# GAMES-UChile/mogptk

Hardware: AMD Instinct MI355X
Metric: log-marginal-likelihood+grad evals/sec, MOSM C=4 N=8192; 1/2/4/8 GPU (higher is better)
Workload: dtype f64

## Files before the change

### mogptk_amd/csrc/exact.hip

```cpp
#include "mogp_model.h"
#include <cstdlib>
#include <limits>

using namespace mogp;

static int wait_stream(hipStream_t st) {
    static const bool spin = !(std::getenv("MOGP_SPIN_WAIT") && std::atoi(std::getenv("MOGP_SPIN_WAIT")) == 0);
    if (!spin) { HIP_TRY(hipStreamSynchronize(st)); return 0; }
    for (;;) {
        const hipError_t e = hipStreamQuery(st);
        if (e == hipSuccess) return 0;
        if (e != hipErrorNotReady) return hip_fail(e, "hipStreamQuery", __FILE__, __LINE__);
    }
}

static hipEvent_t prof_event(mogp_model* m, int idx) {
    if (!m->profiling) return nullptr;
    while ((int)m->ev.size() <= idx) { hipEvent_t e; if (hipEventCreate(&e) != hipSuccess) return nullptr; m->ev.push_back(e); }
    return m->ev[idx];
}

static void kinv_block_ranges(mogp_model* m) {
    std::vector<int> blk;
    tile_blocks(m->sx.off, m->C, blk);
// ... 40 lines not shown
    for (int i = 0; i < nb; ++i) {
        for (int j = 0; j <= i; ++j) {
            if (!need[(size_t)i * nb + j]) continue;
            GemmTask a;
            a.a_off = (int64_t)i * MOGP_TILE; a.b_off = (int64_t)j * MOGP_TILE; a.c_off = (int64_t)i * MOGP_TILE * ld + (int64_t)j * MOGP_TILE;
            a.kt = 4 * MOGP_TILE / 16; a.pad = i + 1;
            acc.push_back(a);
            GemmTask l;
            l.a_off = (int64_t)i * MOGP_TILE * ld + (int64_t)i * MOGP_TILE; l.b_off = (int64_t)i * MOGP_TILE * ld + (int64_t)j * MOGP_TILE;
            l.c_off = a.c_off; l.kt = (int)((ld - (int64_t)i * MOGP_TILE) / 16); l.pad = 0;
            lau.push_back(l);
        }
        prefix[i + 1] = (int)acc.size();
    }
    const double frac = (double)acc.size() / ((double)nb * (nb + 1) / 2);
    m->kinv_fraction = frac;
    if (frac > 0.85) return 0;
    const bool same = acc.size() == m->kinv_acc_tasks.size() && (acc.empty() || std::memcmp(acc.data(), m->kinv_acc_tasks.data(), acc.size() * sizeof(GemmTask)) == 0);
    if (!same || m->d_kinv_acc.n < acc.size()) {
        int rc;
        if ((rc = m->d_kinv_acc.ensure(std::max<size_t>(acc.size(), 1)))) return rc;
        if ((rc = m->d_kinv_lauum.ensure(std::max<size_t>(lau.size(), 1)))) return rc;
        HIP_TRY(hipMemcpyAsync(m->d_kinv_acc.p, acc.data(), acc.size() * sizeof(GemmTask), hipMemcpyHostToDevice, m->st));
        HIP_TRY(hipMemcpyAsync(m->d_kinv_lauum.p, lau.data(), lau.size() * sizeof(GemmTask), hipMemcpyHostToDevice, m->st));
        HIP_TRY(hipStreamSynchronize(m->st));
        m->kinv_acc_tasks.swap(acc); m->kinv_lauum_tasks.swap(lau);
    }
    m->kinv_prefix.swap(prefix);
    m->kinv_sparse = true;
    return 0;
}

static int pin_ensure(mogp_model* m, size_t n) {
    if (n <= m->h_pin_n) return 0;
    if (m->h_pin) { hipError_t e = hipHostFree(m->h_pin); (void)e; m->h_pin = nullptr; m->h_pin_n = 0; }
    HIP_TRY(hipHostMalloc(reinterpret_cast<void**>(&m->h_pin), n * sizeof(double), hipHostMallocDefault));
    m->h_pin_n = n;
    return 0;
}
struct PinLayout {
    size_t nzz, logdet = 0, zz, info, moments, diagG, pivots, total, score, mu, var, fold_info;
    PinLayout(int nb, int64_t Npad, int C, int T, int Wt) : nzz((size_t)((Npad + 3) / 4)) {
        zz = (size_t)nb; info = zz + nzz; moments = info + 1; diagG = moments + (size_t)(C * (C + 1) / 2) * T * Wt; pivots = diagG + C; total = pivots + 2;
        score = total; mu = score + 1; var = mu + (size_t)Npad; fold_info = var + (size_t)Npad;
    }
    explicit PinLayout(const mogp_model* m) : PinLayout(m->nb, m->Npad, m->C, m->T, m->Wt) {}
    size_t held_out_total(bool folds) const { return fold_info + (folds ? 1 : 0); }
};

namespace mogp {
int begin_call(mogp_model* m, int64_t* info, bool one_gpu) {
    m->mean_w = nullptr;
    if (int rc = use_device(m->ctx)) return rc;
    if (info) *info = 0;
    if (one_gpu) one_gpu_call(m);
    return 0;
}

int exact_begin(mogp_model* m, const double* noise_var, const double* data_var, double jitter, GramArgs& ga, double& jabs) {
    const int C = m->C;
    const int64_t N = m->N, Npad = m->Npad;
    if (m->T <= 0) return fail(MOGP_EINVAL, "mogp_model_set_terms must be called before an evaluation");
    if (!noise_var) return fail(MOGP_EINVAL, "noise_var is null");
    { int r__ = ensure_system(m); if (r__) return r__; }
    m->have_W = m->have_Kinv = false;
    m->gemm_ev_used = 0; m->gemm_launches = 0; m->gemm_flops = 0.0;

    double dsum = 0.0;
    if (!m->point_diag.empty()) {
        for (int c = 0; c < C; ++c)
            for (int k = m->sx.off[c]; k < m->sx.off[c + 1]; ++k) dsum += m->point_diag[k] + noise_var[c];
    } else if (m->radial && m->point_kinds) {
        dsum = table_diag_points(m, m->sx);
        for (int c = 0; c < C; ++c) dsum += (double)(m->sx.off[c + 1] - m->sx.off[c]) * noise_var[c];
    } else
    for (int c = 0; c < C; ++c) dsum += (double)(m->sx.off[c + 1] - m->sx.off[c]) * (table_diag(m, c) + noise_var[c]);
    if (data_var) {
        std::vector<double> dv(Npad, 0.0);
        for (int64_t pos = 0; pos < N; ++pos) { dv[pos] = data_var[m->sx.perm[pos]]; dsum += dv[pos]; }
        { int r__ = m->d_dvar.ensure(Npad); if (r__) return r__; }
        HIP_TRY(hipMemcpyAsync(m->d_dvar.p, dv.data(), Npad * sizeof(double), hipMemcpyHostToDevice, m->st));
    }
    jabs = jitter * dsum / (double)N;
    HIP_TRY(hipMemcpyAsync(m->d_noise.p, noise_var, C * sizeof(double), hipMemcpyHostToDevice, m->st));
    static const unsigned long long big = std::numeric_limits<unsigned long long>::max();
    HIP_TRY(hipMemcpyAsync(m->d_info.p, &big, sizeof(big), hipMemcpyHostToDevice, m->st));
    int rc;
    if ((rc = mark(m, 0))) return rc;
    ga = GramArgs{};
    ga.tiles = m->d_tiles.p; ga.xr = m->d_x.p; ga.xc = m->d_x.p; ga.ldxr = ga.ldxc = Npad; ga.nrows = ga.ncols = N;
    if ((rc = m->ph_xx.prepare(m->sx.off, m->sx.off, C, m->T, Npad, Npad, m->st, ga.ph))) return rc;
    ga.table = m->d_table.p; ga.T = m->T; ga.D = m->D; ga.C = C; ga.W = m->Wt;
    ga.out = m->k.A.p; ga.ldo = Npad; ga.noise = m->d_noise.p; ga.dvar = data_var ? m->d_dvar.p : nullptr;
    ga.jitter_abs = jabs; ga.mirror = 0;
    if (m->radial) { ga.kind = m->d_kind.p; ga.shape = m->d_shape.p; }
    return 0;
}
}

namespace mogp { int chain_fallback(mogp_model* m) {
    if (m->flow_ran) {
        m->no_flow = true; m->flow_ran = false;
        m->flow_timeouts++;
        m->flow_retry_at = m->n_fact + m->flow_backoff;
        m->flow_backoff = std::min(m->flow_backoff * 4, 16384);
        for (hipStream_t q : {m->st, m->st2, m->st3, m->st4, m->ctx->st5, m->st_priv}) if (q) HIP_TRY(hipStreamSynchronize(q));
        static bool said_flow = false;
        if (!said_flow) {
            said_flow = true;
            unsigned code = 0;
            if (m->k.flow_flags.p && m->k.flow_cur && m->k.flow_cur->base_err > 0) { hipError_t e = hipMemcpy(&code, m->k.flow_flags.p + m->k.flow_cur->base_err, sizeof(code), hipMemcpyDeviceToHost); (void)e; }
            fprintf(stderr, "mogp: the dataflow kernel timed out (wait 0x%x; GPU shared with another process?); using the stream schedule for the next %d evaluations (said once)\n", code, (int)(m->flow_retry_at - m->n_fact));
            fprintf(stderr, "mogp: the host enqueued that evaluation in %.0f us (longest so far %.0f us)\n", m->flow_enqueue_us, m->flow_enqueue_us_max);
        }
        if (std::getenv("MOGP_FLOW_DEBUG")) { fprintf(stderr, "mogp: dataflow time-out %d of this model\n", m->flow_timeouts); flow_debug_dump(m); }
        return 0;
    }
    if (m->no_chain) return fail(MOGP_EHIP, "chain kernel: a hand-off timed out although the model is on the launch-per-step chain");
    m->no_chain = true;
    for (hipStream_t q : {m->st, m->st2, m->st3, m->st4, m->ctx->st5, m->st_priv}) if (q) HIP_TRY(hipStreamSynchronize(q));
    static bool said = false;
    if (!said) { said = true; fprintf(stderr, "mogp: the persistent chain kernel timed out (GPU shared with another process?); using the launch-per-step chain\n"); }
    return 0;
} }

template <typename F> static int retry_on_streams(mogp_model* m, int rc, F again) {
    if (rc != MOGP_RETRY_NO_CHAIN) return rc;
    if ((rc = chain_fallback(m))) return rc;
    return again();
}

namespace mogp { int report_not_pd(unsigned long long hinfo, int64_t* info) {
    if (info) *info = (int64_t)hinfo;
    return fail(MOGP_ENOTPD, "linalg.cholesky: The factorization could not be completed because the input is not "
                             "positive-definite (the leading minor of order " + std::to_string(hinfo) + " is not positive-definite).");
} }

static int factorize_finish(mogp_model* m, const GramArgs& ga, double* lml, int64_t* info) {
    const int64_t N = m->N, Npad = m->Npad;
    const PinLayout pl(m);
    const unsigned long long big = std::numeric_limits<unsigned long long>::max();
    unsigned long long hinfo = 0;
    std::memcpy(&hinfo, m->h_pin + pl.info, sizeof(hinfo));
    int rc;
    if (hinfo == MOGP_INFO_CHAIN_TIMEOUT) return MOGP_RETRY_NO_CHAIN;
    if (hinfo != big) {
        if (info) *info = (int64_t)hinfo;
        int flag = 0;
        HIP_TRY(hipMemsetAsync(m->d_flag.p, 0, sizeof(int), m->st));
        if ((rc = launch_gram(ga, (int)m->tiles.size(), m->st, m->radial ? m->gate_kinds : 0))) return rc;
        if ((rc = launch_nonfinite_scan(m->k.A.p, Npad, N, m->d_flag.p, m->st))) return rc;
        HIP_TRY(hipMemcpyAsync(&flag, m->d_flag.p, sizeof(int), hipMemcpyDeviceToHost, m->st));
        HIP_TRY(hipStreamSynchronize(m->st));
        if (flag & 1) return fail(MOGP_ENONFINITE, "linalg.cholesky: kernel matrix has NaNs!");
        if (flag & 2) return fail(MOGP_ENONFINITE, "linalg.cholesky: kernel matrix has infinities!");
        return report_not_pd(hinfo, info);
    }
    m->pivot_min = m->h_pin[pl.pivots]; m->pivot_max = m->h_pin[pl.pivots + 1];
    double logdet = 0.0, zz = 0.0;
    for (int i = 0; i < m->nb; ++i) logdet += m->h_pin[pl.logdet + i];
    for (size_t i = 0; i < pl.nzz; ++i) zz += m->h_pin[pl.zz + i];
    if (lml) *lml = -0.5 * (double)N * std::log(2.0 * M_PI) - logdet - 0.5 * zz;
    m->have_W = !m->factor_only && !m->accurate_ran;
    return 0;
}

struct FactorPlan {
    enum Schedule { Fused, Phases, FactorOnly } schedule = Phases;
    bool defer = false;
    bool want_inverse = true;
    bool refine = false;
};

static int factorize(mogp_model* m, const double* noise_var, const double* data_var, double jitter, const FactorPlan& plan,
                     double* lml, double* jitter_abs, int64_t* info, GramArgs* ga_out = nullptr) {
    const bool fuse_inverse = plan.schedule == FactorPlan::Fused, factor_only = plan.schedule == FactorPlan::FactorOnly;
    const int64_t N = m->N, Npad = m->Npad;
    GramArgs ga{};
    double jabs = 0.0;
    int rc = exact_begin(m, noise_var, data_var, jitter, ga, jabs);
    if (rc) return rc;
    if (jitter_abs) *jitter_abs = jabs;
    m->n_fact++;
    if (m->no_flow && m->n_fact >= m->flow_retry_at) m->no_flow = false;
    m->factor_only = factor_only;
    ga.ev0 = prof_event(m, 7); ga.ev1 = prof_event(m, 8);
    m->strip.attach(ga);
    const bool split = fuse_inverse && flow_enabled(m, m->k) && !m->tiles_head.empty() && !m->tiles_tail.empty() && m->st2;
    if (split) {
        GramArgs gh = ga, gt = ga;
        gh.tiles = m->d_tiles_head.p; m->strip_head.attach(gh); gh.ev1 = nullptr;
        gt.tiles = m->d_tiles_tail.p; m->strip_tail.attach(gt); gt.ev0 = nullptr; gt.phases_ready = 1;
        if ((rc = launch_gram(gh, (int)m->tiles_head.size(), m->st, m->radial ? m->gate_kinds : 0))) return rc;
        if ((rc = launch_pad_identity(m->k.A.p, Npad, N, Npad, m->st))) return rc;
        if (!m->gram_ev) HIP_TRY(hipEventCreateWithFlags(&m->gram_ev, hipEventDisableTiming));
        HIP_TRY(hipEventRecord(m->gram_ev, m->st));
        HIP_TRY(hipStreamWaitEvent(m->st2, m->gram_ev, 0));
        if ((rc = launch_gram(gt, (int)m->tiles_tail.size(), m->st2, m->radial ? m->gate_kinds : 0))) return rc;
        if (!m->gram_tail_ev) HIP_TRY(hipEventCreateWithFlags(&m->gram_tail_ev, hipEventDisableTiming));
        HIP_TRY(hipEventRecord(m->gram_tail_ev, m->st2));
        m->k.tail_ready = m->gram_tail_ev;
    } else {
        if ((rc = launch_gram(ga, (int)m->tiles.size(), m->st, m->radial ? m->gate_kinds : 0))) return rc;
        if ((rc = launch_pad_identity(m->k.A.p, Npad, N, Npad, m->st))) return rc;
    }
    ga.ev0 = ga.ev1 = nullptr;
    if ((rc = mark(m, 1))) return rc;

    const PinLayout pl(m);
    if ((rc = pin_ensure(m, pl.total))) return rc;
    if ((rc = m->d_pivots.ensure(2))) return rc;
    if (m->accurate && (rc = m->acc_rhs.ensure((size_t)Npad * MOGP_TILE))) return rc;
    m->k.flow_used = false;
    m->flow_ran = false;
    m->k.want_vec = fuse_inverse;
    m->k.vec_y = m->d_y.p; m->k.vec_z = m->d_z.p; m->k.vec_zz = m->d_zz.p; m->k.vec_part = m->d_alpha.p + Npad;
    const bool accurate = m->accurate && plan.schedule == FactorPlan::Phases;
    m->accurate_ran = accurate;
    m->k.keep_L = m->k.refine_panels = plan.refine || accurate;
    if (factor_only && m->rhs_job && flow_enabled(m, m->k)) rc = spd_potri_flow(m, m->k, m->rhs_job);
    else rc = fuse_inverse ? spd_potri_fused(m, m->k) : spd_potrf(m, m->k);
    m->k.keep_L = m->k.refine_panels = false;
    m->k.want_vec = false; m->k.tail_ready = nullptr;
    if (rc) return rc;
    if ((rc = mark(m, 2))) return rc;
    if (accurate) {
        hipStream_t ms = (plan.want_inverse && m->st2u) ? m->st2u : m->st;
        if (plan.want_inverse) {
            if (ms != m->st) {
                while ((int)m->k.inv_ev.size() < 4) { hipEvent_t e; HIP_TRY(hipEventCreateWithFlags(&e, hipEventDisableTiming)); m->k.inv_ev.push_back(e); }
                HIP_TRY(hipEventRecord(m->k.inv_ev[0], m->st));
                HIP_TRY(hipStreamWaitEvent(ms, m->k.inv_ev[0], 0));
            }
            if ((rc = m->k.Wm.ensure((size_t)Npad * Npad))) return rc;
            HIP_TRY(hipMemsetAsync(m->k.Wm.p, 0, (size_t)Npad * Npad * sizeof(double), ms));
            if ((rc = launch_add_diag(m->k.Wm.p, Npad, Npad, 1.0, ms))) return rc;
            if ((rc = trsm_lower(m, m->k.A.p, Npad, m->nb, m->k.Wm.p, Npad, Npad, false, ms, true))) return rc;
            GemmArgs g{};
            g.A = m->k.Wm.p; g.lda = Npad; g.a_kmajor = 1; g.B = m->k.Wm.p; g.ldb = Npad; g.b_kmajor = 1;
            g.C = m->k.B.p; g.ldc = Npad; g.alpha = 1.0; g.beta = 0.0; g.mode = GM_LAUUM; g.mt = g.nt = m->nb; g.K = (int)Npad;
            if ((rc = gemm_call(m, g, gemm_flops(g, nullptr), ms))) return rc;
            if (ms != m->st) HIP_TRY(hipEventRecord(m->k.inv_ev[1], ms));
        }
        HIP_TRY(hipMemsetAsync(m->acc_rhs.p, 0, (size_t)Npad * MOGP_TILE * sizeof(double), m->st));
        if ((rc = launch_copy2d(m->acc_rhs.p, MOGP_TILE, m->d_y.p, 1, Npad, 1, 1.0, m->st))) return rc;
        if ((rc = trsm_lower(m, m->k.A.p, Npad, m->nb, m->acc_rhs.p, MOGP_TILE, MOGP_TILE, false))) return rc;
        if ((rc = launch_copy2d(m->d_z.p, 1, m->acc_rhs.p, MOGP_TILE, Npad, 1, 1.0, m->st))) return rc;
        HIP_TRY(hipMemsetAsync(m->d_zz.p, 0, pl.nzz * sizeof(double), m->st));
        if ((rc = launch_gemv_rows(m->d_z.p, Npad, 1, Npad, m->d_z.p, m->d_zz.p, m->st))) return rc;
        if ((rc = trsm_lower(m, m->k.A.p, Npad, m->nb, m->acc_rhs.p, MOGP_TILE, MOGP_TILE, true))) return rc;
        if ((rc = launch_copy2d(m->d_alpha.p, 1, m->acc_rhs.p, MOGP_TILE, Npad, 1, 1.0, m->st))) return rc;
        if (plan.want_inverse && ms != m->st) HIP_TRY(hipStreamWaitEvent(m->st, m->k.inv_ev[1], 0));
    } else if (plan.schedule == FactorPlan::Phases && (rc = spd_trtri(m, m->k))) return rc;
    if ((rc = mark(m, 3))) return rc;

    if (factor_only) {
        HIP_TRY(hipMemsetAsync(m->d_zz.p, 0, pl.nzz * sizeof(double), m->st));
    } else if (!accurate) {
        const double* Wp = fuse_inverse ? m->k.Wm.p : m->k.A.p;
        m->w_in_Wm = fuse_inverse;
        if (fuse_inverse && m->k.flow_used && m->k.vec_done) {
            if ((rc = launch_flow_alpha_sum(m->k, m->d_alpha.p, m->st))) return rc;
        } else {
            if ((rc = launch_trmv_lower(Wp, Npad, Npad, m->d_y.p, m->d_z.p, m->d_zz.p, m->st))) return rc;
            if ((rc = launch_trmv_lower_t(Wp, Npad, Npad, m->d_z.p, m->d_alpha.p, m->st))) return rc;
        }
    }
    if (fuse_inverse && (rc = spd_potri_fused_finish(m, m->k))) return rc;
    if ((rc = mark(m, 4))) return rc;
    {
        static const bool fault = std::getenv("MOGP_FLOW_FAULT") && std::atoi(std::getenv("MOGP_FLOW_FAULT")) != 0;
        static const unsigned long long timed_out = MOGP_INFO_CHAIN_TIMEOUT;
        if (fault && m->k.flow_used) HIP_TRY(hipMemcpyAsync(m->d_info.p, &timed_out, sizeof(timed_out), hipMemcpyHostToDevice, m->st));
    }

    const int nzz = (int)pl.nzz;
    if ((rc = launch_pivot_range(m->k.invd.p, N, m->d_pivots.p, m->st))) return rc;
    HIP_TRY(hipMemcpyAsync(m->h_pin + pl.pivots, m->d_pivots.p, 2 * sizeof(double), hipMemcpyDeviceToHost, m->st));
    HIP_TRY(hipMemcpyAsync(m->h_pin + pl.logdet, m->k.logdet.p, m->nb * sizeof(double), hipMemcpyDeviceToHost, m->st));
    constexpr int zz_piece = 2048;
    for (int o = 0; o < nzz; o += zz_piece)
        HIP_TRY(hipMemcpyAsync(m->h_pin + pl.zz + o, m->d_zz.p + o, std::min(zz_piece, nzz - o) * sizeof(double), hipMemcpyDeviceToHost, m->st));
    HIP_TRY(hipMemcpyAsync(m->h_pin + pl.info, m->d_info.p, sizeof(unsigned long long), hipMemcpyDeviceToHost, m->st));
    if (ga_out) *ga_out = ga;
    if (plan.defer) return 0;
    HIP_TRY(hipStreamSynchronize(m->st));
    return factorize_finish(m, ga, lml, info);
}

namespace mogp { void collect_timing(mogp_model* m, int last_mark) {
    if (!m->profiling) return;
    auto el = [&](int a, int b) { float t = 0.f; if (hipEventElapsedTime(&t, m->ev[a], m->ev[b]) != hipSuccess) t = 0.f; return (double)t; };
    std::fill(m->ms, m->ms + MOGP_ST_COUNT, 0.0);
    m->ms[MOGP_ST_GRAM] = el(0, 1);
    m->ms[MOGP_ST_POTRF] = el(1, 2);
    m->ms[MOGP_ST_TRTRI] = el(2, 3);
    m->ms[MOGP_ST_SOLVE] = el(3, 4);
    if (last_mark >= 6) { m->ms[MOGP_ST_LAUUM] = el(4, 5); m->ms[MOGP_ST_MOMENTS] = el(5, 6); }
    m->ms[MOGP_ST_TOTAL] = el(0, last_mark);
    if ((int)m->ev.size() > 8) m->ms[MOGP_ST_GRAM_KERNEL] = el(7, 8);
    if (last_mark >= 6 && (int)m->ev.size() > 10) m->ms[MOGP_ST_MOMENT_KERNEL] = el(9, 10);
    double gsum = 0.0;
    for (size_t i = 0; i + 1 < m->gemm_ev_used; i += 2) {
        float t = 0.f;
        if (hipEventElapsedTime(&t, m->gemm_ev[i], m->gemm_ev[i + 1]) == hipSuccess) gsum += t;
    }
    m->ms[MOGP_ST_GEMM_KERNEL] = gsum;
}

int moment_pass_device(mogp_model* m, const double* kinv, double ksign) {
    const int C = m->C, D = m->D, W = m->Wt, T = m->T, P = C * (C + 1) / 2;
    const int64_t Npad = m->Npad;
    const int rm = m->sh_n > 1 ? m->sh_n : 0;
    const bool own = m->sh_n > 1 && m->own_n == m->sh_n && m->own_rank == m->sh_rank;
    int rc;
    MomentArgs ma{};
    ma.tiles = own ? m->d_tiles_own.p : m->d_tiles.p; ma.ntiles = (int)(own ? m->tiles_own.size() : m->tiles.size());
    ma.x = m->d_x.p; ma.ldx = Npad; ma.nrows = ma.ncols = m->N;
    if ((rc = m->ph_xx.prepare(m->sx.off, m->sx.off, C, T, Npad, Npad, m->st, ma.ph))) return rc;
    ma.table = m->d_table.p; ma.T = T; ma.D = D; ma.C = C; ma.W = W; ma.kinv = kinv; ma.kinv_sign = ksign; ma.ld = Npad; ma.alpha = m->d_alpha.p;
    ma.row_mod = rm; ma.row_rem = m->sh_rank;
    if (m->radial) { ma.kind = m->d_kind.p; ma.shape = m->d_shape.p; }
    ma.partial = m->d_partial.p;
    ma.phases_ready = 1;
    ma.ev0 = prof_event(m, 9); ma.ev1 = prof_event(m, 10);
    if ((rc = launch_moments(ma, m->st, m->radial ? m->gate_kinds : 0))) return rc;
    if ((rc = launch_moment_reduce(m->d_partial.p, own ? m->d_pair_start_own.p : m->d_pair_start.p, P, T, W, D, m->d_moments.p, m->st))) return rc;
    if ((rc = launch_diagG(kinv, Npad, m->d_alpha.p, m->d_chan_off.p, C, m->d_diagG.p, m->st, ksign, rm, m->sh_rank))) return rc;
    if ((rc = mean_grad_enqueue(m, m->d_alpha.p, -1.0))) return rc;
    return mark(m, 6);
}

int moment_pass(mogp_model* m, const double* kinv, double ksign, double* moments, double* diagG) {
    const int C = m->C, W = m->Wt, T = m->T, P = C * (C + 1) / 2;
    int rc;
    if ((rc = moment_pass_device(m, kinv, ksign))) return rc;
    HIP_TRY(hipMemcpyAsync(moments, m->d_moments.p, (size_t)P * T * W * sizeof(double), hipMemcpyDeviceToHost, m->st));
    HIP_TRY(hipMemcpyAsync(diagG, m->d_diagG.p, C * sizeof(double), hipMemcpyDeviceToHost, m->st));
    HIP_TRY(hipStreamSynchronize(m->st));
    return 0;
}

int test_side(mogp_model* m, int64_t S, const double* Xs, const double* kss_diag, int64_t extra_rows, hipStream_t st, TestSide& ts, GramArgs& ga, int R, bool point_diag) {
    const int C = m->C, D = m->D;
    const int64_t Npad = m->Npad;
    SortedX& ss = ts.ss;
    int rc;
    if ((rc = sort_inputs(Xs, S, D, C, MOGP_TILE, ss))) return rc;
    const int64_t Spad = ts.Spad = ss.Mpad, Srow = R * Spad + extra_rows;
    std::vector<GTile> pt;
    build_rect_tiles(ss.off, m->sx.off, C, pt);
    ts.ntiles = (int)pt.size();
    if ((rc = m->d_xs.ensure((size_t)D * Spad))) return rc;
    if ((rc = m->d_Ksf.ensure((size_t)Srow * Npad))) return rc;
    if ((rc = m->d_mu.ensure((size_t)R * Spad))) return rc;
    if ((rc = m->d_kdiag.ensure((size_t)R * Spad))) return rc;
    if ((rc = m->d_ptiles.ensure(std::max<size_t>(pt.size(), 1)))) return rc;
    std::vector<double> kd((size_t)R * Spad, 0.0);
    const bool per_point = point_diag || m->Wt > 2 + 3 * D || (m->radial && m->point_kinds);
    for (int r = 0; r < R; ++r) {
        const double* kr = kss_diag + (size_t)r * (per_point ? S : C);
        for (int c = 0; c < C; ++c)
            for (int pos = ss.off[c]; pos < ss.off[c + 1]; ++pos) kd[(size_t)r * Spad + pos] = per_point ? kr[ss.perm[pos]] : kr[c];
    }
    HIP_TRY(hipMemcpyAsync(m->d_xs.p, ss.xs.data(), (size_t)D * Spad * sizeof(double), hipMemcpyHostToDevice, st));
    HIP_TRY(hipMemcpyAsync(m->d_kdiag.p, kd.data(), (size_t)R * Spad * sizeof(double), hipMemcpyHostToDevice, st));
    HIP_TRY(hipMemcpyAsync(m->d_ptiles.p, pt.data(), pt.size() * sizeof(GTile), hipMemcpyHostToDevice, st));
    HIP_TRY(hipMemsetAsync(m->d_Ksf.p, 0, (size_t)Srow * Npad * sizeof(double), st));
    ga = GramArgs{};
    ga.tiles = m->d_ptiles.p; ga.xr = m->d_xs.p; ga.ldxr = Spad; ga.xc = m->d_x.p; ga.ldxc = Npad; ga.nrows = S; ga.ncols = m->N;
    if ((rc = m->ph_sx.prepare(ss.off, m->sx.off, C, m->T, Spad, Npad, st, ga.ph))) return rc;
    ga.table = m->d_table.p; ga.T = m->T; ga.D = D; ga.C = C; ga.W = m->Wt; ga.out = m->d_Ksf.p; ga.ldo = Npad;
    ga.noise = nullptr; ga.dvar = nullptr; ga.jitter_abs = 0.0; ga.mirror = 0;
    if (m->radial) { ga.kind = m->d_kind.p; ga.shape = m->d_shape.p; }
    return 0;
}
}

static const std::string& grad_path_env() {
    static const std::string grad_path = []() { const char* e = std::getenv("MOGP_GRAD_PATH"); return std::string(e ? e : ""); }();
    return grad_path;
}

static int enqueue_inverse(mogp_model* m, const double* noise_var, const double* data_var, double jitter, bool inverse, bool banded,
                           double* lml, double* jitter_abs, int64_t* info, GramArgs& ga) {
    const std::string& grad_path = grad_path_env();
    int rc;
    if ((rc = ensure_system(m))) return rc;
    if ((rc = kinv_plan(m, inverse && banded && !m->accurate))) return rc;
    const int fused_max = flow_enabled(m, m->k) ? 112 : 80;
    const bool fused = inverse && !m->accurate && (grad_path == "fused" || (grad_path != "phases" && m->nb <= fused_max));
    FactorPlan plan;
    plan.schedule = fused ? FactorPlan::Fused : FactorPlan::Phases; plan.defer = inverse; plan.want_inverse = inverse;
    if ((rc = factorize(m, noise_var, data_var, jitter, plan, lml, jitter_abs, info, &ga))) return rc;
    if (!inverse) return 0;
    if (!fused && !m->accurate_ran && (rc = spd_lauum(m, m->k))) return rc;
    return mark(m, 5);
}

static int grad_enqueue(mogp_model* m, const PinLayout& pl) {
    HIP_TRY(hipMemcpyAsync(m->h_pin + pl.moments, m->d_moments.p, (pl.diagG - pl.moments) * sizeof(double), hipMemcpyDeviceToHost, m->st));
    HIP_TRY(hipMemcpyAsync(m->h_pin + pl.diagG, m->d_diagG.p, m->C * sizeof(double), hipMemcpyDeviceToHost, m->st));
    return 0;
}
static void grad_finish(mogp_model* m, const double* diagG, double* trG) {
    double tr = 0.0;
    for (int c = 0; c < m->C; ++c) tr += diagG[c];
    *trG = tr;
    mean_grad_collect(m);
    collect_timing(m, 6);
}
static void grad_collect(mogp_model* m, const PinLayout& pl, double* moments, double* diagG, double* trG) {
    std::memcpy(moments, m->h_pin + pl.moments, (pl.diagG - pl.moments) * sizeof(double));
    std::memcpy(diagG, m->h_pin + pl.diagG, m->C * sizeof(double));
    grad_finish(m, diagG, trG);
}

static int held_out_eval(mogp_model* m, const double* noise_var, const double* data_var, double jitter, int flags, const int32_t* fold, int64_t nfolds,
                         double* score, double* mu, double* var, double* moments, double* diagG, double* trG, double* jitter_abs, int64_t* info) {
    const bool grad = (flags & MOGP_EVAL_GRAD) != 0, folds = fold != nullptr;
    int rc;
    if ((rc = begin_call(m, info, true))) return rc;
    auto again = [&]() {
        return folds ? mogp_exact_cv(m, noise_var, data_var, jitter, flags, fold, nfolds, score, mu, var, moments, diagG, trG, jitter_abs, info)
                     : mogp_exact_loo(m, noise_var, data_var, jitter, flags, score, mu, var, moments, diagG, trG, jitter_abs, info);
    };
    if ((rc = ensure_system(m))) return rc;
    if ((rc = folds ? cv_workspace(m, fold, nfolds, grad) : loo_workspace(m, grad))) return rc;
    const PinLayout pl(m);
    if ((rc = pin_ensure(m, pl.held_out_total(folds)))) return rc;
    const int64_t N = m->N, Npad = m->Npad;
    GramArgs ga{};
    if ((rc = enqueue_inverse(m, noise_var, data_var, jitter, true, false, nullptr, jitter_abs, info, ga))) return retry_on_streams(m, rc, again);
    if ((rc = held_out_points(m, m->k.B.p, folds, grad))) return rc;
    if (grad) {
        m->have_W = false;
        if ((rc = held_out_adjoint(m, m->k.B.p, m->k.A.p, folds))) return rc;
        if ((rc = loo_moment_pass(m))) return rc;
        if ((rc = grad_enqueue(m, pl))) return rc;
    }
    const double* v = m->loo.vec.p;
    double* h = m->h_pin;
    HIP_TRY(hipMemcpyAsync(h + pl.score, v + LOO_SUM * Npad, sizeof(double), hipMemcpyDeviceToHost, m->st));
    HIP_TRY(hipMemcpyAsync(h + pl.mu, v + LOO_MU * Npad, N * sizeof(double), hipMemcpyDeviceToHost, m->st));
    HIP_TRY(hipMemcpyAsync(h + pl.var, v + LOO_VAR * Npad, N * sizeof(double), hipMemcpyDeviceToHost, m->st));
    if (folds) HIP_TRY(hipMemcpyAsync(h + pl.fold_info, m->d_info.p, sizeof(unsigned long long), hipMemcpyDeviceToHost, m->st));
    if ((rc = wait_stream(m->st))) return rc;
    if ((rc = factorize_finish(m, ga, nullptr, info))) return retry_on_streams(m, rc, again);
    if (grad) m->have_W = false;
    if (folds) {
        unsigned long long finfo = 0;
        std::memcpy(&finfo, h + pl.fold_info, sizeof(finfo));
        if (finfo != std::numeric_limits<unsigned long long>::max()) {
            if (info) *info = (int64_t)(finfo - 1) / 256;
            return fail(MOGP_ENOTPD, "mogp_exact_cv: the block of Kj^-1 over fold " + std::to_string((finfo - 1) / 256) + " is not positive definite (pivot " +
                                     std::to_string((finfo - 1) % 256 + 1) + " of its factorisation): Kj is too ill-conditioned for this fold");
        }
        for (int64_t pos = 0; pos < N; ++pos)
            if (m->cv.label[pos] < 0) h[pl.mu + pos] = h[pl.var + pos] = std::numeric_limits<double>::quiet_NaN();
    }
    *score = h[pl.score];
    scatter_by_perm(m->sx, h + pl.mu, mu);
    scatter_by_perm(m->sx, h + pl.var, var);
    m->have_Kinv = true;
    m->kinv_in_A = false;
    if (!grad) { collect_timing(m, 5); return MOGP_OK; }
    grad_collect(m, pl, moments, diagG, trG);
    return MOGP_OK;
}

extern "C" {

int mogp_exact_eval(mogp_model* m, const double* noise_var, const double* data_var, double jitter, int flags,
                    double* lml, double* moments, double* diagG, double* trG, double* jitter_abs, int64_t* info) {
    if (!m) return fail(MOGP_EINVAL, "mogp_exact_eval: model is null");
    int rc;
    if ((rc = begin_call(m, info, true))) return rc;
    const std::string& grad_path = grad_path_env();
    const bool sweep = grad_path == "sweep" && (flags & MOGP_EVAL_GRAD);
    const bool grad = (flags & MOGP_EVAL_GRAD) != 0;
    GramArgs ga{};
    auto again = [&]() { return mogp_exact_eval(m, noise_var, data_var, jitter, flags, lml, moments, diagG, trG, jitter_abs, info); };
    if (grad && (!moments || !diagG || !trG)) return fail(MOGP_EINVAL, "mogp_exact_eval: gradient outputs are null");
    if (sweep) {
        if ((rc = ensure_system(m))) return rc;
// ... 324 lines not shown
```

### mogptk_amd/csrc/flow.hip

```cpp
#include "mogp_model.h"
#include <unistd.h>
#include <chrono>
#include <set>

#include <cstdio>
#include <cstdlib>

namespace mogp {

typedef double d4_t __attribute__((ext_vector_type(4)));
typedef double d2_t __attribute__((ext_vector_type(2)));

#define FL_BK 16
#define FL_ROWK 18
#define FL_WTM 4
#define FL_WTN 2
#define FL_NWJ 4
#define FL_NWI 2
#define FL_NT 512
#define FL_COLK (MOGP_TILE + 16)
#define FL_OPER (MOGP_TILE * FL_ROWK)
#define FL_LDS_DOUBLES (2 * 2 * FL_OPER)
#define FL_LDS_BYTES (FL_LDS_DOUBLES * 8 + 16 + 3 * 64 * 4 + 16)
static_assert(MOGP_TILE * FL_ROWK == 16 * FL_COLK, "one LDS operand slot serves both layouts");
// ... 620 lines not shown
            vec.push_back(t);
        }
        for (int jg = 0; jg * 4 < k1(b); ++jg) {
            FlowTask t = mk(b, PH_APART, 32 | 1, nk(b));
            t.ar = (uint16_t)k0(b); t.br = (uint16_t)b; t.ac = (uint16_t)jg;
            dep(t, ZR(b), (unsigned)nk(b));
            vec.push_back(t);
        }
    }
    std::vector<const std::vector<FlowTask>*> order = {&q[Q_LOOK2], &q[Q_SEMI], &q[Q_INVCRIT], &vec};
    for (int d = 2; d < no + 3; ++d) {
        if (d < no && !into[d].empty()) order.push_back(&into[d]);
        if (d - 3 >= 0 && d - 3 < no && !trail[d - 3].empty()) order.push_back(&trail[d - 3]);
    }
    order.push_back(rhs_nt > 0 ? &rrest : &acc);
    for (size_t k = order.size(); k-- > 1;) if (order[k]->empty()) order.erase(order.begin() + (long)k);
    if ((int)order.size() > FLOW_MAXQ) {
        std::vector<FlowTask> rest;
        std::vector<const std::vector<FlowTask>*> tail(order.begin() + (FLOW_MAXQ - 2), order.end() - 1);
        for (auto* v : tail) rest.insert(rest.end(), v->begin(), v->end());
        std::stable_sort(rest.begin(), rest.end(), [](const FlowTask& x, const FlowTask& y) { return x.key < y.key; });
        p.folded = rest;
        order.erase(order.begin() + (FLOW_MAXQ - 2), order.end() - 1);
        order.insert(order.end() - 1, &p.folded);
    }
    p.nq = (int)order.size();
    for (int qi = 0; qi < p.nq; ++qi) {
        p.qbase[qi] = (int)p.tasks.size(); p.qsize[qi] = (int)order[qi]->size();
        p.tasks.insert(p.tasks.end(), order[qi]->begin(), order[qi]->end());
    }
    p.flops = 2.0 * MOGP_TILE * MOGP_TILE * FL_BK * tiles_k;
}

__global__ void k_alpha_sum(const double* __restrict__ part, int64_t npad, int no, int ob, double* __restrict__ out) {
    const int64_t col = (int64_t)blockIdx.x * blockDim.x + threadIdx.x;
    if (col >= npad) return;
    double s = 0.0;
    for (int r = (int)(col / MOGP_TILE) / ob; r < no; ++r) s += part[(int64_t)r * npad + col];
    out[col] = s;
}
int launch_flow_alpha_sum(const Spd& w, double* alpha, hipStream_t st) {
    const FlowPlan& p = w.flow_cur ? *w.flow_cur : w.flow;
    hipLaunchKernelGGL(k_alpha_sum, dim3((unsigned)((w.Npad + 255) / 256)), dim3(256), 0, st, w.vec_part, w.Npad, p.nouter, p.ob, alpha);
    HIP_TRY(hipGetLastError());
    return 0;
}

bool flow_enabled(const mogp_model* m, const Spd& w) {
    const char* eo = std::getenv("MOGP_FLOW");
    const char* en = std::getenv("MOGP_FLOW_MIN");
    const int on = eo ? std::atoi(eo) : 1, nmin = en ? std::atoi(en) : 8;
    if (!on || (m->no_flow && m->n_fact < m->flow_retry_at) || !chain_enabled(m) || !m->ctx->st_priv) return false;
    if (m->kinv_sparse && &w == &m->k) return false;
    return w.nb >= nmin && w.nb <= 0xfff0;
}

int spd_potri_flow(mogp_model* m, Spd& w, const FlowRhs* rhs) {
    const int nb = w.nb, ob = 4;
    const int64_t ld = w.Npad;
    int rc;
    const auto host_t0 = std::chrono::steady_clock::now();
    hipStream_t crit = m->st, priv = m->st_priv, bulk = m->st2;
    if (w.Wm.n < (size_t)ld * ld) {
        if ((rc = w.Wm.ensure((size_t)ld * ld))) return rc;
        HIP_TRY(hipMemsetAsync(w.Wm.p, 0, (size_t)ld * ld * sizeof(double), crit));
    }
    if ((rc = w.Lm.ensure((size_t)ld * ld))) return rc;
    if (!rhs && (rc = w.Wt.ensure((size_t)ld * ld))) return rc;
    const bool replay = m->replay_flow && !rhs && &w == &m->k;
    FlowPlan& plan = rhs ? w.flow_rhs : replay ? w.flow_replay : w.flow;
    DevBuf<FlowTask>& d_tasks = rhs ? w.flow_tasks_rhs : replay ? w.flow_tasks_replay : w.flow_tasks;
    DevBuf<int>& d_qmeta = rhs ? w.flow_qmeta_rhs : replay ? w.flow_qmeta_replay : w.flow_qmeta;
    const int rhs_nt = rhs ? rhs->nt : 0;
    if (plan.nb != nb || plan.ob != ob || plan.rhs_nt != rhs_nt) {
        flow_build(nb, ob, plan, rhs_nt, replay);
        if ((rc = d_tasks.ensure(plan.tasks.size()))) return rc;
        if ((rc = d_qmeta.ensure(2 * FLOW_MAXQ))) return rc;
        int qm[2 * FLOW_MAXQ] = {0};
        for (int q = 0; q < plan.nq; ++q) { qm[2 * q] = plan.qbase[q]; qm[2 * q + 1] = plan.qsize[q]; }
        HIP_TRY(hipStreamSynchronize(crit));
        HIP_TRY(dev_upload(d_tasks.p, plan.tasks.data(), plan.tasks.size() * sizeof(FlowTask)));
        HIP_TRY(dev_upload(d_qmeta.p, qm, sizeof(qm)));
    }
    if ((rc = w.flow_flags.ensure((size_t)plan.nflags))) return rc;
    if (!w.flow_diag.p) {
        if ((rc = w.flow_diag.ensure(FLOW_DIAG_WORDS))) return rc;
        HIP_TRY(hipMemsetAsync(w.flow_diag.p, 0, FLOW_DIAG_WORDS * sizeof(unsigned), crit));
    }
    w.flow_cur = &plan;
    const FlowPlan& p = plan;
    const int nouter = p.nouter;
    if ((rc = w.chain_flags.ensure((size_t)(nouter + 1) * MOGP_CHAIN_FLAGS))) return rc;
    HIP_TRY(hipMemsetAsync(w.chain_flags.p, 0, (size_t)(nouter + 1) * MOGP_CHAIN_FLAGS * sizeof(unsigned), crit));
    HIP_TRY(hipMemsetAsync(w.flow_flags.p, 0, (size_t)p.nflags * sizeof(unsigned), crit));
    if (replay) {
        std::vector<unsigned> preset((size_t)p.nflags, 0u);
        for (const FlowPlan::Chain& c : p.chain) preset[c.done_idx] = c.expect;
        HIP_TRY(hipMemcpyAsync(w.flow_flags.p, preset.data(), preset.size() * sizeof(unsigned), hipMemcpyHostToDevice, crit));
        HIP_TRY(hipStreamSynchronize(crit));
    }
    if (!rhs && w.want_vec && w.vec_zz) HIP_TRY(hipMemsetAsync(w.vec_zz, 0, (size_t)((ld + 3) / 4) * sizeof(double), crit));
    static const bool want_trace = std::getenv("MOGP_FLOW_TRACE") && std::atoi(std::getenv("MOGP_FLOW_TRACE")) != 0;
    if (want_trace) {
        if ((rc = w.flow_trace.ensure(FLOW_TRACE_W * p.tasks.size() + 4 * (size_t)nouter))) return rc;
        HIP_TRY(hipMemsetAsync(w.flow_trace.p, 0, w.flow_trace.n * sizeof(unsigned long long), crit));
    }
    while ((int)w.inv_ev.size() < 4) {
        hipEvent_t e;
        HIP_TRY(hipEventCreateWithFlags(&e, hipEventDisableTiming));
        w.inv_ev.push_back(e);
    }
    hipEvent_t start = w.inv_ev[0], e_flow = w.inv_ev[1], e_chain = w.inv_ev[2];
    HIP_TRY(hipEventRecord(start, crit));
    HIP_TRY(hipStreamWaitEvent(bulk, start, 0));
    HIP_TRY(hipStreamWaitEvent(priv, start, 0));

    static std::atomic<unsigned long long> attr_done{0ull};
    static std::atomic<unsigned long long> attr_done_dbg{0ull};
    { int r__ = set_max_dynamic_lds(reinterpret_cast<const void*>(k_flow<false>), FL_LDS_BYTES, attr_done); if (r__) return r__; }
    { int r__ = set_max_dynamic_lds(reinterpret_cast<const void*>(k_flow<true>), FL_LDS_BYTES, attr_done_dbg); if (r__) return r__; }
    static const int wg_per_cu = std::getenv("MOGP_FLOW_WGS") ? std::max(1, std::atoi(std::getenv("MOGP_FLOW_WGS"))) : 2;
    int cus = (m->ctx->ncu > 0 ? m->ctx->ncu : 256) - m->ctx->ncu_reserved;
    { static const int drop = std::getenv("MOGP_FLOW_DROP_CUS") ? std::atoi(std::getenv("MOGP_FLOW_DROP_CUS")) : 16;
      if (drop > 0 && drop < cus) cus -= drop; }
    FlowArgs g{};
    g.bA = w.A.p; g.bL = w.Lm.p; g.bWt = rhs ? rhs->T : w.Wt.p; g.bWm = w.Wm.p; g.bB = rhs ? rhs->X : w.B.p; g.ld = ld;
    g.tasks = d_tasks.p; g.qmeta = d_qmeta.p; g.flags = w.flow_flags.p;
    g.nq = p.nq; g.ncas = FLOW_NCAS; g.base_heads = p.base_heads; g.base_err = p.base_err; g.info = m->d_info.p;
    g.trace = want_trace ? w.flow_trace.p : nullptr;
    g.diag = w.flow_diag.p;
    static const bool want_post = std::getenv("MOGP_FLOW_DEBUG") && std::atoi(std::getenv("MOGP_FLOW_DEBUG")) != 0;
    if (want_post) {
        const size_t nwg = (size_t)wg_per_cu * ((size_t)cus + (size_t)m->ctx->ncu_reserved);
        if ((rc = w.flow_post.ensure(nwg * FLOW_POST_W))) return rc;
        HIP_TRY(hipMemsetAsync(w.flow_post.p, 0, w.flow_post.n * sizeof(unsigned), bulk));
        g.post = w.flow_post.p;
        if ((rc = w.flow_done.ensure(p.tasks.size()))) return rc;
        HIP_TRY(hipMemsetAsync(w.flow_done.p, 0, p.tasks.size(), bulk));
        g.done = w.flow_done.p;
    }
    g.npad = ld;
    { const char* e = std::getenv("MOGP_FLOW_REFILL"); g.refill = e ? std::atoi(e) : 0; }
    { const char* e = std::getenv("MOGP_FLOW_CLAIM1"); g.claim_one = e ? std::atoi(e) : 0; }
    { const char* e = std::getenv("MOGP_FLOW_NHI"); g.nhi = e ? std::atoi(e) : 0; }
    { const char* e = std::getenv("MOGP_FLOW_NAP"); g.nap_max = e ? (unsigned)std::max(0, std::atoi(e)) : 4u; }
    { const char* e = std::getenv("MOGP_FLOW_NAP_CALM"); g.nap_calm = e ? (unsigned)std::max(0, std::atoi(e)) : 0u; if (g.nap_calm < g.nap_max) g.nap_calm = g.nap_max; }
    w.vec_done = false;
    if (!rhs && w.want_vec && w.vec_y && w.vec_z && w.vec_zz && w.vec_part) {
        g.vy = w.vec_y; g.vz = w.vec_z; g.vzz = w.vec_zz; g.vpart = w.vec_part;
        w.vec_done = true;
    }
    hipEvent_t pe0 = nullptr, pe1 = nullptr;
    if (m->profiling) {
        if (m->gemm_ev_used + 2 > m->gemm_ev.size())
            for (int i = 0; i < 64; ++i) { hipEvent_t e; HIP_TRY(hipEventCreate(&e)); m->gemm_ev.push_back(e); }
        pe0 = m->gemm_ev[m->gemm_ev_used++]; pe1 = m->gemm_ev[m->gemm_ev_used++];
        HIP_TRY(hipEventRecord(pe0, bulk));
    }
    if (rhs && rhs->ready) HIP_TRY(hipStreamWaitEvent(bulk, rhs->ready, 0));
    const bool dbg_kernel = g.post != nullptr || g.trace != nullptr;
    static_assert(sizeof(FlowArgs) <= 512, "Spd::flow_args slots");
    if ((rc = w.flow_args.ensure(1024))) return rc;
    if (w.flow_args_h.size() != 2048) w.flow_args_h.assign(2048, (char)0xff);
    auto upload = [&](size_t slot, const FlowArgs& a, hipStream_t st) -> int {
        char* held = w.flow_args_h.data() + slot;
        char* fresh_ = w.flow_args_h.data() + 1024 + slot;
        std::memset(fresh_, 0, 512);
        std::memcpy(fresh_, &a, sizeof(a));
        if (std::memcmp(held, fresh_, 512) == 0) return 0;
        HIP_TRY(hipStreamSynchronize(st));
        HIP_TRY(dev_upload(w.flow_args.p + slot, fresh_, 512));
        std::memcpy(held, fresh_, 512);
        return 0;
    };
    if ((rc = upload(0, g, bulk))) return rc;
    const FlowArgs* d_g = reinterpret_cast<const FlowArgs*>(w.flow_args.p);
    FlowHot hot{};
    hot.bA = g.bA; hot.bL = g.bL; hot.bWt = g.bWt; hot.bWm = g.bWm; hot.bB = g.bB; hot.ld = g.ld; hot.tasks = g.tasks; hot.qmeta = g.qmeta; hot.flags = g.flags;
    hot.nq = g.nq; hot.ncas = g.ncas; hot.base_heads = g.base_heads; hot.base_err = g.base_err; hot.nap_max = g.nap_max; hot.nap_calm = g.nap_calm;
    if (dbg_kernel) hipLaunchKernelGGL(k_flow<true>, dim3(wg_per_cu * cus), dim3(FL_NT), FL_LDS_BYTES, bulk, d_g, hot);
    else hipLaunchKernelGGL(k_flow<false>, dim3(wg_per_cu * cus), dim3(FL_NT), FL_LDS_BYTES, bulk, d_g, hot);
    HIP_TRY(hipGetLastError());
    if (pe1) HIP_TRY(hipEventRecord(pe1, bulk));
    HIP_TRY(hipEventRecord(e_flow, bulk));
    m->gemm_launches += 1;
    m->gemm_flops += p.flops;

    unsigned* ferr = w.flow_flags.p + p.base_err;
    for (int kb = 0; kb < nouter && !replay; ++kb) {
        const int k0 = kb * ob, k1 = std::min(k0 + ob, nb), nk = k1 - k0, na = std::min(ob, nb - k1);
        const FlowPlan::Chain& pc = p.chain[kb];
        ChainFlow cf{};
        cf.done_flag = w.flow_flags.p + pc.done_idx; cf.write_through = 1;
        cf.trace = want_trace ? w.flow_trace.p + FLOW_TRACE_W * p.tasks.size() + 4 * (size_t)kb : nullptr;
        cf.diag = w.flow_diag.p;
        if ((rc = launch_chain(w.A.p, ld, k0, nk, w.invd.p, w.logdet.p, m->d_info.p, 0, w.Wm.p + (int64_t)k0 * MOGP_TILE * (ld + 1), ld,
                               w.chain_flags.p + (size_t)kb * MOGP_CHAIN_FLAGS, ferr, priv, &cf))) return rc;
        if (na <= 0) continue;
        GemmArgs t1{};
        t1.A = w.A.p + (int64_t)k1 * MOGP_TILE * ld + (int64_t)k0 * MOGP_TILE; t1.lda = ld; t1.a_kmajor = 0;
        t1.B = w.Wm.p + (int64_t)k0 * MOGP_TILE * (ld + 1); t1.ldb = ld; t1.b_kmajor = 0;
        t1.C = w.Lm.p + (int64_t)k1 * MOGP_TILE * ld + (int64_t)k0 * MOGP_TILE; t1.ldc = ld; t1.alpha = 1.0; t1.beta = 0.0;
        t1.mode = GM_KHI_J; t1.small = 1; t1.mt = 2 * na; t1.nt = nk; t1.K = nk * MOGP_TILE;
        t1.fl_flags = w.flow_flags.p; t1.fl_nwait = pc.t1_nwait;
        for (int k = 0; k < pc.t1_nwait; ++k) { t1.fl_widx[k] = pc.t1_widx[k]; t1.fl_wval[k] = pc.t1_wval[k]; }
        static const unsigned hook_spins = std::getenv("MOGP_FLOW_HOOK_SPINS") ? (unsigned)std::atoll(std::getenv("MOGP_FLOW_HOOK_SPINS")) : 0u;
        t1.fl_spins = hook_spins; t1.fl_diag = w.flow_diag.p;
        t1.fl_wt = 1; t1.fl_sig = 1; t1.fl_sig_base = pc.t1_sig_base; t1.fl_sig_shift = 1; t1.fl_err = ferr; t1.sk_info = m->d_info.p;
        if ((rc = launch_gemm(t1, priv))) return rc;
        if (kb == 0 && w.tail_ready) HIP_TRY(hipStreamWaitEvent(priv, w.tail_ready, 0));
        GemmArgs t2{};
        t2.A = t1.C; t2.lda = ld; t2.a_kmajor = 0; t2.B = t1.C; t2.ldb = ld; t2.b_kmajor = 0;
        t2.C = w.A.p + (int64_t)k1 * MOGP_TILE * (ld + 1); t2.ldc = ld; t2.alpha = -1.0; t2.beta = 1.0;
        t2.mode = GM_RECT_LOWER; t2.small = 2; t2.mt = 2 * na; t2.nt = 2 * na; t2.K = nk * MOGP_TILE;
        t2.fl_flags = w.flow_flags.p; t2.fl_nwait = pc.t2_wval ? 1 : 0; t2.fl_widx[0] = pc.t2_widx; t2.fl_wval[0] = pc.t2_wval;
        t2.fl_err = ferr; t2.sk_info = m->d_info.p; t2.fl_spins = hook_spins; t2.fl_diag = w.flow_diag.p;
        if ((rc = launch_gemm(t2, priv))) return rc;
        m->gemm_flops += gemm_flops(t1, nullptr) + gemm_flops(t2, nullptr);
    }
    static const bool tail_on = !(std::getenv("MOGP_FLOW_TAIL") && std::atoi(std::getenv("MOGP_FLOW_TAIL")) == 0);
    if (tail_on && m->ctx->ncu_reserved > 0 && !replay) {
        if (rhs && rhs->ready) HIP_TRY(hipStreamWaitEvent(priv, rhs->ready, 0));
        g.post_base = wg_per_cu * cus;
        if ((rc = upload(512, g, priv))) return rc;
        const FlowArgs* d_g2 = reinterpret_cast<const FlowArgs*>(w.flow_args.p + 512);
        if (dbg_kernel) hipLaunchKernelGGL(k_flow<true>, dim3(wg_per_cu * m->ctx->ncu_reserved), dim3(FL_NT), FL_LDS_BYTES, priv, d_g2, hot);
        else hipLaunchKernelGGL(k_flow<false>, dim3(wg_per_cu * m->ctx->ncu_reserved), dim3(FL_NT), FL_LDS_BYTES, priv, d_g2, hot);
        HIP_TRY(hipGetLastError());
    }
    HIP_TRY(hipEventRecord(e_chain, priv));
    HIP_TRY(hipStreamWaitEvent(crit, e_flow, 0));
    HIP_TRY(hipStreamWaitEvent(crit, e_chain, 0));
    w.fused_last_inv = nullptr; w.fused_last_wt = nullptr;
    w.flow_used = true;
    m->flow_ran = true;
    m->flow_enqueue_us = std::chrono::duration<double, std::micro>(std::chrono::steady_clock::now() - host_t0).count();
    m->flow_enqueue_us_max = std::max(m->flow_enqueue_us_max, m->flow_enqueue_us);
    { const char* e = std::getenv("MOGP_FLOW_DEBUG");
      if (e && std::atoi(e) == 2 && &w == &m->k) { usleep(60000); fprintf(stderr, "mogp: dataflow state 60 ms after the evaluation was enqueued\n"); flow_debug_dump(m); } }
    return 0;
}

}

namespace mogp { void flow_debug_dump(mogp_model* m) {
    if (!m->k.flow_flags.p || !m->k.flow_cur) return;
    const FlowPlan& p = *m->k.flow_cur;
    std::vector<unsigned> fl((size_t)p.nflags);
    hipError_t e = hipMemcpy(fl.data(), m->k.flow_flags.p, fl.size() * sizeof(unsigned), hipMemcpyDeviceToHost); (void)e;
    std::vector<unsigned long long> tr;
    if (m->k.flow_trace.p && m->k.flow_trace.n >= FLOW_TRACE_W * p.tasks.size()) {
        tr.resize(FLOW_TRACE_W * p.tasks.size());
        e = hipMemcpy(tr.data(), m->k.flow_trace.p, tr.size() * sizeof(unsigned long long), hipMemcpyDeviceToHost); (void)e;
    }
    fprintf(stderr, "  error word 0x%x\n", fl[p.base_err]);
    std::set<unsigned> holders;
    for (int q = 0; q < p.nq; ++q) {
        const unsigned h = fl[p.base_heads + q];
        const unsigned claimed = std::min<unsigned>(h, (unsigned)p.qsize[q]);
        unsigned done = 0, shown = 0;
        fprintf(stderr, "  queue %2d: head %u of %d", q, h, p.qsize[q]);
        for (unsigned hh = 0; hh < (unsigned)p.qsize[q]; ++hh) {
            const size_t ti = (size_t)p.qbase[q] + hh;
            const FlowTask& t = p.tasks[ti];
            const bool fin = !tr.empty() && tr[FLOW_TRACE_W * ti + 4] != 0;
            if (fin) { ++done; continue; }
            if (tr.empty() && hh + 4 < claimed) continue;
            if (hh > claimed || shown >= 6) continue;
            ++shown;
            fprintf(stderr, "\n      %s task %u key %u C(buf %d %d,%d) A(buf %d %d,%d) B(buf %d %d,%d) kt %d var %d:", hh < claimed ? "CLAIMED" : "head   ", hh, t.key,
                    t.cbuf, t.cr, t.cc, t.abuf, t.ar, t.ac, t.bbuf, t.br, t.bc, t.kt, t.var);
            for (int d = 0; d < t.ndep; ++d) fprintf(stderr, " flag[%u]=%u/%u", t.dep[d], fl[t.dep[d]], (unsigned)t.need[d]);
            if (!tr.empty()) {
                const unsigned long long w5 = tr[FLOW_TRACE_W * ti + 5];
                if (w5 >> 63) { fprintf(stderr, "  (HELD by wg %llu%s)", w5 & 0xffff, tr[FLOW_TRACE_W * ti + 1] ? ": STARTED, not finished" : ""); holders.insert((unsigned)(w5 & 0xffff)); }
                else fprintf(stderr, "  (taken by wg %llu: %s)", w5 & 0xffff, tr[FLOW_TRACE_W * ti + 1] ? "running" : "not started");
            }
        }
        if (!tr.empty()) fprintf(stderr, "\n      finished %u", done);
        fprintf(stderr, "\n");
// ... 182 lines not shown
```

### mogptk_amd/csrc/gram.hip

```cpp
#include "mogp_internal.h"

#include <algorithm>
#include <vector>
#include <cstdlib>

#ifdef MOGP_GRAM_DEBUG
#define GRAM_DBG(a, bit) ((a).dbg & (bit))
#else
#define GRAM_DBG(a, bit) 0
#endif

namespace mogp {

typedef double d2_t __attribute__((ext_vector_type(2)));

__device__ __forceinline__ double frac_turn(double p) { return p - rint(p); }

#define GT_SKIP (-1)
#define GT_GENERAL 0
#define GT_SKIP_EXPONENT 50.0
#define GT_DEGREE(zmax) ((zmax) <= 1.19e-3 ? 4 : (zmax) <= 4.93e-3 ? 5 : (zmax) <= 0.0139 ? 6 : (zmax) <= 0.0308 ? 7 : (zmax) <= 0.0578 ? 8 : (zmax) <= 0.0968 ? 9 : \
                         (zmax) <= 0.149 ? 10 : (zmax) <= 0.2147 ? 11 : (zmax) <= 0.294 ? 12 : 14)
#define GT_DEGREE_CASES(X) X(4) X(5) X(6) X(7) X(8) X(9) X(10) X(11) X(12) X(14)

__device__ __forceinline__ double fast_exp(double x) {
    const double n = rint(x * 1.44269504088896338700e+00);
    double r = fma(-n, 6.93147180369123816490e-01, x);
    r = fma(-n, 1.90821492927058770002e-10, r);
    double p = 1.6059043836821613e-10;
    p = fma(p, r, 2.08767569878681e-09);
    p = fma(p, r, 2.505210838544172e-08);
    p = fma(p, r, 2.755731922398589e-07);
    p = fma(p, r, 2.7557319223985893e-06);
    p = fma(p, r, 2.48015873015873e-05);
    p = fma(p, r, 1.984126984126984e-04);
    p = fma(p, r, 1.388888888888889e-03);
    p = fma(p, r, 8.333333333333333e-03);
    p = fma(p, r, 4.1666666666666664e-02);
    p = fma(p, r, 1.6666666666666666e-01);
    p = fma(p, r, 0.5);
    p = fma(p, r, 1.0);
    p = fma(p, r, 1.0);
    return ldexp(p, (int)n);
}

template <int N>
__device__ __forceinline__ double exp_taylor(double z) {
    constexpr double c[15] = {1.0, 1.0, 0.5, 1.6666666666666666e-01, 4.1666666666666664e-02, 8.333333333333333e-03,
                              1.388888888888889e-03, 1.984126984126984e-04, 2.48015873015873e-05, 2.7557319223985893e-06,
                              2.755731922398589e-07, 2.505210838544172e-08, 2.08767569878681e-09, 1.6059043836821613e-10,
                              1.1470745597729725e-11};
    double p = c[N];
#pragma unroll
    for (int k = N - 1; k >= 0; --k) p = fma(p, z, c[k]);
    return p;
}

struct PhaseArgs {
    const double* x; int64_t ld; const int* off; const double* table; int T, D, C, W, role; double* cs; double* sn;
};
__global__ __launch_bounds__(256) void k_phase_table(PhaseArgs a) {
    const int64_t pt = (int64_t)blockIdx.x * 256 + threadIdx.x;
    if (pt >= a.off[a.C]) return;
    const int o = blockIdx.y, t = blockIdx.z, D = a.D, W = a.W;
    int c = 0;
    while (pt >= a.off[c + 1]) ++c;
    const int pair = a.role == 0 ? c * a.C + o : o * a.C + c;
    const double* row = a.table + ((size_t)pair * a.T + t) * W;
    double ph = a.role == 0 ? row[1] : 0.0;
    for (int d = 0; d < D; ++d) {
        const double m = row[2 + D + d], xv = a.x[(size_t)d * a.ld + pt];
        ph = a.role == 0 ? fma(m, xv + row[2 + 2 * D + d], ph) : fma(m, xv, ph);
    }
    double sn, cs;
    sincospi(2.0 * frac_turn(ph), &sn, &cs);
    const size_t idx = ((size_t)o * a.T + t) * a.ld + pt;
    a.cs[idx] = cs;
    a.sn[idx] = sn;
}

struct CentreArgs { const double* x; int64_t ld; const int* off; int C, D; double* cen; double* half; };
__global__ __launch_bounds__(64) void k_block_centres(CentreArgs a) {
    int b = blockIdx.x, c = 0;
    for (; c < a.C; ++c) {
        const int nb = (a.off[c + 1] - a.off[c] + MOGP_GT - 1) / MOGP_GT;
        if (b < nb) break;
        b -= nb;
    }
    if (c >= a.C) return;
    const int start = a.off[c] + b * MOGP_GT, n = min(MOGP_GT, a.off[c + 1] - start), lane = threadIdx.x;
    for (int d = 0; d < a.D; ++d) {
        const double v = a.x[(size_t)d * a.ld + start + (lane < n ? lane : 0)];
        double lo = v, hi = v;
#pragma unroll
        for (int off = 32; off > 0; off >>= 1) { lo = fmin(lo, __shfl_xor(lo, off, 64)); hi = fmax(hi, __shfl_xor(hi, off, 64)); }
        if (lane == 0) { a.cen[(size_t)d * a.ld + start] = 0.5 * (lo + hi); a.half[(size_t)d * a.ld + start] = 0.5 * (hi - lo); }
    }
}

size_t phase_ws_doubles(int C, int T, int64_t ldr, int64_t ldc) { return (size_t)2 * (C * T + MOGP_MAXD) * (size_t)(ldr + ldc); }

struct PhaseView {
    const double *rcs, *rsn, *ccs, *csn, *rcen, *rhalf, *ccen, *chalf;
};
__host__ __device__ static inline PhaseView phase_view(double* ws, int C, int T, int D, int64_t ldr, int64_t ldc) {
    PhaseView v;
    double* p = ws;
    v.rcs = p; p += (size_t)C * T * ldr; v.rsn = p; p += (size_t)C * T * ldr;
    v.ccs = p; p += (size_t)C * T * ldc; v.csn = p; p += (size_t)C * T * ldc;
    v.rcen = p; p += (size_t)D * ldr; v.rhalf = p; p += (size_t)D * ldr;
    v.ccen = p; p += (size_t)D * ldc; v.chalf = p;
    return v;
}

static int launch_phase_tables(const PhaseRef& ph, const double* xr, int64_t ldxr, int64_t nr, const double* xc, int64_t ldxc, int64_t nc,
                               const double* table, int T, int D, int C, int W, hipStream_t s) {
    if (!ph.ws || !ph.offr || !ph.offc) { set_error("Gram / moment launch without a phase workspace"); return -1; }
    const PhaseView v = phase_view(ph.ws, C, T, D, ldxr, ldxc);
    PhaseArgs a;
    a.table = table; a.T = T; a.D = D; a.C = C; a.W = W;
    a.x = xr; a.ld = ldxr; a.off = ph.offr; a.role = 0; a.cs = const_cast<double*>(v.rcs); a.sn = const_cast<double*>(v.rsn);
    if (nr > 0) hipLaunchKernelGGL(k_phase_table, dim3((unsigned)((nr + 255) / 256), C, T), dim3(256), 0, s, a);
    a.x = xc; a.ld = ldxc; a.off = ph.offc; a.role = 1; a.cs = const_cast<double*>(v.ccs); a.sn = const_cast<double*>(v.csn);
    if (nc > 0) hipLaunchKernelGGL(k_phase_table, dim3((unsigned)((nc + 255) / 256), C, T), dim3(256), 0, s, a);
    CentreArgs c;
    c.C = C; c.D = D;
    c.x = xr; c.ld = ldxr; c.off = ph.offr; c.cen = const_cast<double*>(v.rcen); c.half = const_cast<double*>(v.rhalf);
    if (nr > 0) hipLaunchKernelGGL(k_block_centres, dim3((unsigned)((nr + MOGP_GT - 1) / MOGP_GT + C)), dim3(64), 0, s, c);
    c.x = xc; c.ld = ldxc; c.off = ph.offc; c.cen = const_cast<double*>(v.ccen); c.half = const_cast<double*>(v.chalf);
    if (nc > 0) hipLaunchKernelGGL(k_block_centres, dim3((unsigned)((nc + MOGP_GT - 1) / MOGP_GT + C)), dim3(64), 0, s, c);
    HIP_TRY(hipGetLastError());
    return 0;
}

template <int DM>
struct TileLds {
    double cu[MOGP_TC][MOGP_GT], su[MOGP_TC][MOGP_GT], cw[MOGP_TC][MOGP_GT], sw[MOGP_TC][MOGP_GT];
    double V[MOGP_TC][DM], s[MOGP_TC][DM], M[MOGP_TC][DM], A[MOGP_TC];
    double Kp[MOGP_TC][DM];
    double L[MOGP_TC][DM], e[MOGP_TC][DM];
    int deg[MOGP_TC];
};
template <int DM>
struct TileCtx { double cr[DM], cc[DM], hr[DM], hc[DM]; };

template <int DM>
__device__ __forceinline__ void tile_centres(TileCtx<DM>& X, const GTile& tl, int D, const PhaseView& v, int64_t ldxr, int64_t ldxc) {
    for (int d = 0; d < D; ++d) {
        X.cr[d] = v.rcen[(size_t)d * ldxr + tl.r0]; X.hr[d] = v.rhalf[(size_t)d * ldxr + tl.r0];
        X.cc[d] = v.ccen[(size_t)d * ldxc + tl.c0]; X.hc[d] = v.chalf[(size_t)d * ldxc + tl.c0];
    }
}

template <int DM>
__device__ __forceinline__ void tile_context(TileCtx<DM>& X, double (&p)[4][DM], double (&q)[4][DM], const GTile& tl, int D,
                                             const PhaseView& v, const double* __restrict__ xr, int64_t ldxr,
                                             const double* __restrict__ xc, int64_t ldxc, int rg, int cg) {
    tile_centres<DM>(X, tl, D, v, ldxr, ldxc);
#pragma unroll
    for (int m = 0; m < 4; ++m)
        for (int d = 0; d < D; ++d) {
            p[m][d] = xr[(size_t)d * ldxr + tl.r0 + min(rg * 4 + m, tl.nr - 1)] - X.cr[d];
            q[m][d] = xc[(size_t)d * ldxc + tl.c0 + min(cg * 4 + m, tl.nc - 1)] - X.cc[d];
        }
}

constexpr int STAGE_ITEMS = MOGP_TC * MOGP_GT * 2 / 256;
template <int DM>
struct StageItem { double x[DM], cs, sn; };

template <int DM>
__device__ __forceinline__ void stage_item_load(StageItem<DM>& I, int which, int t, int pnt, const GTile& tl, int D, int C, int T, int t0,
                                                const PhaseView& v, const double* __restrict__ xr, int64_t ldxr,
                                                const double* __restrict__ xc, int64_t ldxc) {
    const int i = tl.pair / C, j = tl.pair - i * C;
    if (which == 0) {
        const int64_t g = tl.r0 + min(pnt, tl.nr - 1);
        const size_t k = ((size_t)j * T + t0 + t) * ldxr + g;
        I.cs = v.rcs[k]; I.sn = v.rsn[k];
        for (int d = 0; d < D; ++d) I.x[d] = xr[(size_t)d * ldxr + g];
    } else {
        const int64_t g = tl.c0 + min(pnt, tl.nc - 1);
        const size_t k = ((size_t)i * T + t0 + t) * ldxc + g;
        I.cs = v.ccs[k]; I.sn = v.csn[k];
        for (int d = 0; d < D; ++d) I.x[d] = xc[(size_t)d * ldxc + g];
    }
}

template <int DM, bool AMP, bool RAD = false, int GATE = 0, bool SPLIT = true>
__device__ __forceinline__ void stage_item_compute(TileLds<DM>& L, const StageItem<DM>& I, const TileCtx<DM>& X, const double* tab, int W,
                                                   int which, int t, int pnt, int D, int t0, const int* kinds = nullptr) {
    const double* row = tab + (size_t)(t0 + t) * W;
    const double A = row[0];
    if constexpr (RAD) {
        const int kd = kinds[t0 + t] & MOGP_KIND_MASK;
        const bool per = kd == MOGP_KIND_PERIODIC, dot = kd == MOGP_KIND_DOT;
        const int deg = (AMP && A == 0.0 && !dot) ? GT_SKIP : GT_GENERAL;
        if (pnt == 0 && which == 0) {
            L.deg[t] = deg; L.A[t] = A;
            for (int d = 0; d < D; ++d) {
                L.V[t][d] = row[2 + d]; L.M[t][d] = row[2 + D + d];
                L.s[t][d] = (X.cr[d] - X.cc[d]) + row[2 + 2 * D + d];
                L.Kp[t][d] = X.cr[d]; L.L[t][d] = X.cc[d];
            }
            L.e[t][0] = row[1];
        }
        if (deg == GT_SKIP) return;
        if (dot) return;
        if (GATE > 1 && (kd == MOGP_KIND_WDOT || kd == MOGP_KIND_WHITE)) return;
        if (GATE && kd == MOGP_KIND_GATE) {
            const double z = row[2] * (I.x[0] - row[2 + D]);
            const double e = exp(-fabs(z)), r = 1.0 / (1.0 + e);
            const double h = z >= 0.0 ? r : e * r, hc = z >= 0.0 ? e * r : r;
// ... 680 lines not shown
            const int deg = __builtin_amdgcn_readfirstlane(L.deg[u3][t]);
            if (deg == GT_SKIP || GRAM_DBG(a, 2)) continue;
            const double V = L.tab[t][1], s = L.s[u3][t];
            double cu[4], su[4], cw[4], sw[4];
#pragma unroll
            for (int m = 0; m < 4; ++m) { cu[m] = L.cu[b][t][rg * 4 + m]; su[m] = L.su[b][t][rg * 4 + m]; }
#pragma unroll
            for (int n = 0; n < 4; ++n) { cw[n] = L.cw[b][t][SL::cs(cg * 4 + n)]; sw[n] = L.sw[b][t][SL::cs(cg * 4 + n)]; }
            switch (deg) {
                #define GT_CASE(N) case N: strip_term<N, 4>(acc, p, q, V, s, cu, su, cw, sw); break;
                GT_DEGREE_CASES(GT_CASE)
#undef GT_CASE
                default: strip_term<0, 4>(acc, p, q, V, s, cu, su, cw, sw); break;
            }
        }
        if (u + 2 < sg.n) {
            col_commit(b);
            scalars(u + 2, cc_n, hc_n);
        }
        cc0 = cc1; cc1 = cc_n;
        if (sg.diag && u + 1 == sg.n) {
#pragma unroll
            for (int m = 0; m < 4; ++m) {
                const int lr = rg * 4 + m;
                const int64_t r = sg.r0 + lr;
#pragma unroll
                for (int n = 0; n < 4; ++n) {
                    const int lc = cg * 4 + n;
                    if (lc > lr) continue;
                    double val = acc[m][n];
                    if (a.noise != nullptr && lc == lr) {
                        val += a.noise[ci] + a.jitter_abs;
                        if (a.dvar != nullptr) val += a.dvar[r];
                    }
                    a.out[r * a.ldo + c0 + lc] = val;
                    if (a.out2) a.out2[r * a.ldo + c0 + lc] = val;
                }
            }
        } else if (!(GRAM_DBG(a, 1) && acc[0][0] != 12345.678)) {
            double* o = a.out + (int64_t)(sg.r0 + rg * 4) * a.ldo + c0 + cg * 4;
#pragma unroll
            for (int m = 0; m < 4; ++m) {
                *reinterpret_cast<d2_t*>(o + m * a.ldo) = (d2_t){acc[m][0], acc[m][1]};
                *reinterpret_cast<d2_t*>(o + m * a.ldo + 2) = (d2_t){acc[m][2], acc[m][3]};
            }
            if (a.out2) {
                double* o2 = a.out2 + (int64_t)(sg.r0 + rg * 4) * a.ldo + c0 + cg * 4;
#pragma unroll
                for (int m = 0; m < 4; ++m) {
                    *reinterpret_cast<d2_t*>(o2 + m * a.ldo) = (d2_t){acc[m][0], acc[m][1]};
                    *reinterpret_cast<d2_t*>(o2 + m * a.ldo + 2) = (d2_t){acc[m][2], acc[m][3]};
                }
            }
        }
        asm volatile("s_waitcnt lgkmcnt(0)\n\ts_barrier" ::: "memory");
        if (u + 3 < sg.n) col_fetch(c0 + 3 * MOGP_GT);
    }
}

void split_strip_tiles(const std::vector<GTile>& tiles, int maxrun, std::vector<GSeg>& segs, std::vector<GTile>& rest) {
    segs.clear(); rest.clear();
    for (const GTile& t : tiles) {
        const bool fast = t.nr == MOGP_GT && t.nc == MOGP_GT && (t.c0 & 1) == 0;
        if (!fast) { rest.push_back(t); continue; }
        const int dg = (t.flags & GT_DIAG) ? 1 : 0;
        if (!segs.empty()) {
            GSeg& g = segs.back();
            if (!g.diag && g.pair == t.pair && g.r0 == t.r0 && g.c0 + g.n * MOGP_GT == t.c0 && g.n < maxrun) { ++g.n; g.diag = dg; continue; }
        }
        segs.push_back(GSeg{t.r0, t.c0, 1, t.pair, dg, {0, 0, 0}});
    }
}

int launch_gram(const GramArgs& a0, int ntiles, hipStream_t s, int rows) {
    if (ntiles <= 0) return 0;
    GramArgs a = a0;
    if (a.W <= 0) a.W = 2 + 3 * a.D;
#ifdef MOGP_GRAM_DEBUG
    static const int dbg = []() { const char* e = std::getenv("MOGP_GRAM_DBG"); return e ? std::atoi(e) : 0; }();
    a.dbg = dbg;
#else
    a.dbg = 0;
#endif
    int rc = a.phases_ready ? 0 : launch_phase_tables(a.ph, a.xr, a.ldxr, a.nrows, a.xc, a.ldxc, a.ncols, a.table, a.T, a.D, a.C, a.W, s);
    if (rc) return rc;
    static const int ncu = []() { int dev = 0; hipDeviceProp_t pr; if (hipGetDevice(&dev) != hipSuccess || hipGetDeviceProperties(&pr, dev) != hipSuccess) return 256; return pr.multiProcessorCount; }();
    const int grid = std::min(ntiles, 2 * ncu);
    const size_t tab_bytes = (size_t)a.C * a.C * a.T * a.W * sizeof(double);
    a.tab_lds = tab_bytes <= 24 * 1024;
    const size_t dyn = a.tab_lds ? tab_bytes : 0;
    if (a.ev0) HIP_TRY(hipEventRecord(a.ev0, s));
    if (a.kind) {
        if (!a.shape) { set_error("launch_gram: kinds without shapes"); return -1; }
        if (a.W != 2 + 3 * a.D) { set_error("launch_gram: radial profiles do not combine with enveloped term rows"); return -1; }
        if (rows == 1 && a.D != 1) { set_error("launch_gram: gate rows take one input dimension"); return -1; }
        if (rows == 1) {
            hipLaunchKernelGGL((k_gram<1, true, 1>), dim3(grid), dim3(256), dyn, s, a, ntiles);
        } else if (rows > 1) {
        switch (a.D) {
            case 1: hipLaunchKernelGGL((k_gram<1, true, 2>), dim3(grid), dim3(256), dyn, s, a, ntiles); break;
            case 2: hipLaunchKernelGGL((k_gram<2, true, 2>), dim3(grid), dim3(256), dyn, s, a, ntiles); break;
            case 3: hipLaunchKernelGGL((k_gram<3, true, 2>), dim3(grid), dim3(256), dyn, s, a, ntiles); break;
            default: hipLaunchKernelGGL((k_gram<0, true, 2>), dim3(grid), dim3(256), dyn, s, a, ntiles); break;
        }
        } else {
        switch (a.D) {
            case 1: hipLaunchKernelGGL((k_gram<1, true>), dim3(grid), dim3(256), dyn, s, a, ntiles); break;
            case 2: hipLaunchKernelGGL((k_gram<2, true>), dim3(grid), dim3(256), dyn, s, a, ntiles); break;
            case 3: hipLaunchKernelGGL((k_gram<3, true>), dim3(grid), dim3(256), dyn, s, a, ntiles); break;
            default: hipLaunchKernelGGL((k_gram<0, true>), dim3(grid), dim3(256), dyn, s, a, ntiles); break;
        }
        }
        if (a.ev1) HIP_TRY(hipEventRecord(a.ev1, s));
        HIP_TRY(hipGetLastError());
        return 0;
    }
    if (a.segs && a.nsegs > 0 && a.D == 1 && a.W == 5 && a.T <= GS_TC_MAX && !a.mirror && (a.ldo & 1) == 0) {
        if (a.T <= 4) hipLaunchKernelGGL((k_gram_strip2<4>), dim3(a.nsegs), dim3(256), 0, s, a, a.segs);
        else hipLaunchKernelGGL((k_gram_strip2<8>), dim3(a.nsegs), dim3(256), 0, s, a, a.segs);
        if (a.nrest > 0) {
            a.tiles = a.rest;
            hipLaunchKernelGGL(k_gram<1>, dim3(std::min(a.nrest, 2 * ncu)), dim3(256), dyn, s, a, a.nrest);
        }
        if (a.ev1) HIP_TRY(hipEventRecord(a.ev1, s));
        HIP_TRY(hipGetLastError());
        return 0;
    }
    switch (a.D) {
        case 1: hipLaunchKernelGGL(k_gram<1>, dim3(grid), dim3(256), dyn, s, a, ntiles); break;
        case 2: hipLaunchKernelGGL(k_gram<2>, dim3(grid), dim3(256), dyn, s, a, ntiles); break;
        case 3: hipLaunchKernelGGL(k_gram<3>, dim3(grid), dim3(256), dyn, s, a, ntiles); break;
        default: hipLaunchKernelGGL(k_gram<0>, dim3(grid), dim3(256), dyn, s, a, ntiles); break;
    }
    if (a.ev1) HIP_TRY(hipEventRecord(a.ev1, s));
    HIP_TRY(hipGetLastError());
    return 0;
}

template <int DM, int DB, bool ENV>
__device__ __forceinline__ void dx_term(double (&acc)[DB][4][4], const double (&p)[4][DM], const double (&q)[4][DM],
                                        const TileLds<DM>& L, int t, int D, int d0,
                                        const double (&cu)[4], const double (&su)[4], const double (&cw)[4], const double (&sw)[4]) {
    const double* V = L.V[t];
    const double* s = L.s[t];
    const double* Mv = L.M[t];
#pragma unroll
    for (int m = 0; m < 4; ++m) {
        __builtin_amdgcn_sched_barrier(0);
#pragma unroll
        for (int n = 0; n < 4; ++n) {
            const double e = gauss_general<DM>(p[m], q[n], V, s, L.L[t], L.e[t], D);
            const double kc = e * fma(cu[m], cw[n], su[m] * sw[n]);
            const double ks = e * fma(su[m], cw[n], -cu[m] * sw[n]);
            for (int d = 0; d < D; ++d) {
                if (d < d0 || d >= d0 + DB) continue;
                const double u = (p[m][d] - q[n][d]) + s[d];
                double j = -fma(V[d] * u, kc, 6.283185307179586476925286766559 * Mv[d] * ks);
                if (ENV) j = fma(-0.5 * L.L[t][d] * (0.5 * (p[m][d] + q[n][d]) + L.e[t][d]), kc, j);
#pragma unroll
                for (int dd = 0; dd < DB; ++dd) acc[dd][m][n] += (d - d0 == dd) ? j : 0.0;
            }
        }
    }
}

template <int DM, int DB, bool WT>
__device__ __forceinline__ void dx_term_radial(double (&acc)[DB][4][4], const double (&w)[4][4], const double (&p)[4][DM], const double (&q)[4][DM],
// ... 81 lines not shown

    for (int d0 = 0; d0 < D; d0 += DB) {
        double acc[DB][4][4];
#pragma unroll
        for (int dd = 0; dd < DB; ++dd)
#pragma unroll
            for (int m = 0; m < 4; ++m)
#pragma unroll
                for (int n = 0; n < 4; ++n) acc[dd][m][n] = 0.0;
        for (int t0 = 0, nt; t0 < a.T; t0 += nt) {
            if constexpr (RAD) nt = radial_chunk(a.kind, a.T, t0); else nt = min(MOGP_TC, a.T - t0);
            if (t0 > 0 || d0 > 0) __syncthreads();
            stage_chunk<DM, true, false, RAD, 0, false>(L, X, tl, tab, W, D, a.C, a.T, t0, nt, v, a.xr, a.ldxr, a.xc, a.ldxc, tid, kinds);
            __syncthreads();
            if constexpr (RAD) {
                const int* kd = kinds + t0;
                const double* sh = a.shape + (size_t)tl.pair * a.T + t0;
                for (int t = 0, te; t < nt; t = te + 1) {
                    bool skip = false;
                    for (te = t;; ++te) {
                        skip |= L.deg[te] == GT_SKIP;
                        if (te == nt - 1 || !(__builtin_amdgcn_readfirstlane(kd[te]) & MOGP_KIND_TIMES)) break;
                    }
                    if (skip) continue;
                    if (te == t) {
                        dx_term_radial<DM, DB, false>(acc, one, p, q, L, t, D, d0, __builtin_amdgcn_readfirstlane(kd[t]) & MOGP_KIND_MASK, sh[t], rg, cg);
                        continue;
                    }
                    for (int h = t; h <= te; ++h) {
                        double prod[4][4];
#pragma unroll
                        for (int m = 0; m < 4; ++m)
#pragma unroll
                            for (int n = 0; n < 4; ++n) prod[m][n] = 1.0;
                        for (int f = t; f <= te; ++f)
                            if (f != h) group_factor_radial<DM, true, 0>(prod, p, q, L, f, D, __builtin_amdgcn_readfirstlane(kd[f]) & MOGP_KIND_MASK, sh[f], rg, cg);
                        dx_term_radial<DM, DB, true>(acc, prod, p, q, L, h, D, d0, __builtin_amdgcn_readfirstlane(kd[h]) & MOGP_KIND_MASK, sh[h], rg, cg);
                    }
                }
            } else {
                for (int t = 0; t < nt; ++t) {
                    if (L.deg[t] == GT_SKIP) continue;
                    double cu[4], su[4], cw[4], sw[4];
#pragma unroll
                    for (int m = 0; m < 4; ++m) {
                        cu[m] = L.cu[t][rg * 4 + m]; su[m] = L.su[t][rg * 4 + m];
                        cw[m] = L.cw[t][cg * 4 + m]; sw[m] = L.sw[t][cg * 4 + m];
                    }
                    dx_term<DM, DB, ENV>(acc, p, q, L, t, D, d0, cu, su, cw, sw);
                }
            }
        }
#pragma unroll
        for (int dd = 0; dd < DB; ++dd) {
            if (d0 + dd >= D) continue;
            double* out = a.out + (int64_t)(d0 + dd) * dstride;
#pragma unroll
            for (int m = 0; m < 4; ++m) {
                const int lr = rg * 4 + m;
                if (lr >= tl.nr) continue;
                double* o = out + (int64_t)(tl.r0 + lr) * a.ldo + tl.c0 + cg * 4;
                if (full) {
                    *reinterpret_cast<d2_t*>(o) = (d2_t){acc[dd][m][0], acc[dd][m][1]};
                    *reinterpret_cast<d2_t*>(o + 2) = (d2_t){acc[dd][m][2], acc[dd][m][3]};
                } else {
#pragma unroll
                    for (int n = 0; n < 4; ++n)
                        if (cg * 4 + n < tl.nc) o[n] = acc[dd][m][n];
                }
            }
        }
    }
}

int launch_gram_dx(const GramArgs& a0, int ntiles, int64_t dstride, hipStream_t s) {
    if (ntiles <= 0) return 0;
    GramArgs a = a0;
    if (a.W <= 0) a.W = 2 + 3 * a.D;
    a.dbg = 0; a.tab_lds = 0;
    if (a.D < 1 || a.D > MOGP_MAXD) { set_error("launch_gram_dx: input dimension out of range"); return -1; }
    const bool env = a.W > 2 + 3 * a.D;
    if (a.kind && (!a.shape || env)) { set_error("launch_gram_dx: kinds without shapes, or with enveloped term rows"); return -1; }
    if (a.W != 2 + 3 * a.D && a.W != 2 + 5 * a.D) { set_error("launch_gram_dx: table rows of an unknown width"); return -1; }
    int rc = a.phases_ready ? 0 : launch_phase_tables(a.ph, a.xr, a.ldxr, a.nrows, a.xc, a.ldxc, a.ncols, a.table, a.T, a.D, a.C, a.W, s);
    if (rc) return rc;
    if (a.ev0) HIP_TRY(hipEventRecord(a.ev0, s));
#define DX_LAUNCH(DT, ENV, RAD) hipLaunchKernelGGL((k_gram_dx<DT, ENV, RAD>), dim3(ntiles), dim3(256), 0, s, a, ntiles, dstride)
    if (a.kind) {
        switch (a.D) {
            case 1: DX_LAUNCH(1, false, true); break;
            case 2: DX_LAUNCH(2, false, true); break;
            case 3: DX_LAUNCH(3, false, true); break;
            default: DX_LAUNCH(0, false, true); break;
        }
    } else if (env) {
        switch (a.D) {
            case 1: DX_LAUNCH(1, true, false); break;
            case 2: DX_LAUNCH(2, true, false); break;
            case 3: DX_LAUNCH(3, true, false); break;
            default: DX_LAUNCH(0, true, false); break;
        }
    } else {
        switch (a.D) {
            case 1: DX_LAUNCH(1, false, false); break;
            case 2: DX_LAUNCH(2, false, false); break;
            case 3: DX_LAUNCH(3, false, false); break;
            default: DX_LAUNCH(0, false, false); break;
        }
    }
#undef DX_LAUNCH
    if (a.ev1) HIP_TRY(hipEventRecord(a.ev1, s));
    HIP_TRY(hipGetLastError());
    return 0;
}


__device__ __forceinline__ void radial_profile3(int kind, double shape, double s, double& phi, double& psi, double& chi) {
    s = fmax(s, 0.0);
    switch (kind) {
        case MOGP_KIND_RQ: {
            const double b = fma(s, 0.5 / shape, 1.0), ib = 1.0 / b;
            phi = exp(-shape * log(b));
            psi = phi * ib;
            chi = ((shape + 1.0) / shape) * psi * ib;
        } break;
        case MOGP_KIND_MATERN32: {
            const double r = sqrt(3.0 * s), e = exp(-r);
            phi = fma(r, e, e);
            psi = 3.0 * e;
            chi = r > 0.0 ? 9.0 * e / r : 0.0;
        } break;
        case MOGP_KIND_MATERN52: {
            const double r = sqrt(5.0 * s), e = exp(-r);
            phi = fma(r, r, 3.0 * (1.0 + r)) * (e * (1.0 / 3.0));
            psi = (5.0 / 3.0) * fma(r, e, e);
            chi = (25.0 / 3.0) * e;
        } break;
        case MOGP_KIND_SINC: {
            const double x = 9.869604401089358 * s;
            if (x <= 1.0) {
                double a = 2.8114572543455206e-15;
                a = fma(-x, a, 7.6471637318198164e-13);
                a = fma(-x, a, 1.6059043836821613e-10);
                a = fma(-x, a, 2.505210838544172e-08);
                a = fma(-x, a, 2.7557319223985893e-06);
                a = fma(-x, a, 1.984126984126984e-04);
                a = fma(-x, a, 8.333333333333333e-03);
                a = fma(-x, a, 1.6666666666666666e-01);
                phi = fma(-x, a, 1.0);
                double b = 4.4983316069528329e-14;
                b = fma(-x, b, 1.0706029224547743e-11);
                b = fma(-x, b, 1.9270852604185937e-09);
                b = fma(-x, b, 2.505210838544172e-07);
                b = fma(-x, b, 2.2045855379188714e-05);
                b = fma(-x, b, 1.1904761904761906e-03);
                b = fma(-x, b, 3.3333333333333333e-02);
                b = fma(-x, b, 3.3333333333333331e-01);
                psi = 9.869604401089358 * b;
                double c = 3.5231792294250488e-18;
                c = fma(-x, c, 1.1837882210868172e-15);
                c = fma(-x, c, 3.1487144778081596e-13);
                c = fma(-x, c, 6.4236175347286462e-11);
                c = fma(-x, c, 9.6354263020929683e-09);
                c = fma(-x, c, 1.0020843354176688e-06);
                c = fma(-x, c, 6.6137566137566142e-05);
                c = fma(-x, c, 2.3809523809523812e-03);
                c = fma(-x, c, 3.3333333333333333e-02);
// ... 145 lines not shown
            for (int n = 0; n < 4; ++n) acc[m][n] = 0.0;
        for (int t0 = 0, nt; t0 < a.T; t0 += nt) {
            if constexpr (RAD) nt = radial_chunk(a.kind, a.T, t0); else nt = min(MOGP_TC, a.T - t0);
            if (t0 > 0 || de > 0) __syncthreads();
            stage_chunk<DM, true, false, RAD, 0, false>(L, X, tl, tab, W, D, a.C, a.T, t0, nt, v, a.xr, a.ldxr, a.xc, a.ldxc, tid, kinds);
            __syncthreads();
            if constexpr (RAD) {
                const int* kd = kinds + t0;
                const double* sh = a.shape + (size_t)tl.pair * a.T + t0;
                for (int t = 0, te; t < nt; t = te + 1) {
                    bool skip = false;
                    for (te = t;; ++te) {
                        skip |= L.deg[te] == GT_SKIP;
                        if (te == nt - 1 || !(__builtin_amdgcn_readfirstlane(kd[te]) & MOGP_KIND_TIMES)) break;
                    }
                    if (skip) continue;
#pragma unroll 1
                    for (int m = 0; m < 4; ++m) {
                        double pm[DM], P[4], Pa[4], Pb[4], Pab[4];
#pragma unroll
                        for (int j = 0; j < DM; ++j) {
                            pm[j] = 0.0;
#pragma unroll
                            for (int mm = 0; mm < 4; ++mm) pm[j] = fma(p[mm][j], mm == m ? 1.0 : 0.0, pm[j]);
                        }
                        dxdx_row_radial<DM>(P, Pa, Pb, Pab, pm, q, L, t, D, d, e, __builtin_amdgcn_readfirstlane(kd[t]) & MOGP_KIND_MASK, sh[t], rg * 4 + m, cg);
                        for (int h = t + 1; h <= te; ++h) {
                            double k[4], ka[4], kb[4], kab[4];
                            dxdx_row_radial<DM>(k, ka, kb, kab, pm, q, L, h, D, d, e, __builtin_amdgcn_readfirstlane(kd[h]) & MOGP_KIND_MASK, sh[h], rg * 4 + m, cg);
#pragma unroll
                            for (int n = 0; n < 4; ++n) {
                                Pab[n] = fma(Pab[n], k[n], fma(Pa[n], kb[n], fma(Pb[n], ka[n], P[n] * kab[n])));
                                Pa[n] = fma(Pa[n], k[n], P[n] * ka[n]);
                                Pb[n] = fma(Pb[n], k[n], P[n] * kb[n]);
                                P[n] *= k[n];
                            }
                        }
#pragma unroll
                        for (int mm = 0; mm < 4; ++mm)
#pragma unroll
                            for (int n = 0; n < 4; ++n) acc[mm][n] += mm == m ? Pab[n] : 0.0;
                    }
                }
            } else {
                for (int t = 0; t < nt; ++t) {
                    if (L.deg[t] == GT_SKIP) continue;
                    double cu[4], su[4], cw[4], sw[4];
#pragma unroll
                    for (int m = 0; m < 4; ++m) {
                        cu[m] = L.cu[t][rg * 4 + m]; su[m] = L.su[t][rg * 4 + m];
                        cw[m] = L.cw[t][cg * 4 + m]; sw[m] = L.sw[t][cg * 4 + m];
                    }
                    dxdx_term<DM, ENV>(acc, p, q, L, t, D, d, e, cu, su, cw, sw);
                }
            }
        }
        double* out = a.out + ((int64_t)d * bstride) * a.ldo + (int64_t)e * bstride;
        double* outT = a.out + ((int64_t)e * bstride) * a.ldo + (int64_t)d * bstride;
#pragma unroll
        for (int m = 0; m < 4; ++m) {
            const int lr = rg * 4 + m;
            if (lr >= tl.nr) continue;
#pragma unroll
            for (int n = 0; n < 4; ++n) {
                const int lc = cg * 4 + n;
                if (lc >= tl.nc) continue;
                out[(int64_t)(tl.r0 + lr) * a.ldo + tl.c0 + lc] = acc[m][n];
                if (mirror) outT[(int64_t)(tl.c0 + lc) * a.ldo + tl.r0 + lr] = acc[m][n];
            }
        }
    }
}

int launch_gram_dxdx(const GramArgs& a0, int ntiles, int64_t bstride, hipStream_t s) {
    if (ntiles <= 0) return 0;
    GramArgs a = a0;
    if (a.W <= 0) a.W = 2 + 3 * a.D;
    a.dbg = 0; a.tab_lds = 0;
    if (a.D < 1 || a.D > MOGP_MAXD) { set_error("launch_gram_dxdx: input dimension out of range"); return -1; }
    const bool env = a.W > 2 + 3 * a.D;
    if (a.kind && (!a.shape || env)) { set_error("launch_gram_dxdx: kinds without shapes, or with enveloped term rows"); return -1; }
    if (a.W != 2 + 3 * a.D && a.W != 2 + 5 * a.D) { set_error("launch_gram_dxdx: table rows of an unknown width"); return -1; }
    if (a.xc != a.xr || a.ldxc != a.ldxr || a.ldo < a.D * bstride) { set_error("launch_gram_dxdx: not a symmetric launch, or the output is too narrow for D blocks"); return -1; }
    int rc = a.phases_ready ? 0 : launch_phase_tables(a.ph, a.xr, a.ldxr, a.nrows, a.xc, a.ldxc, a.ncols, a.table, a.T, a.D, a.C, a.W, s);
    if (rc) return rc;
    if (a.ev0) HIP_TRY(hipEventRecord(a.ev0, s));
#define DXDX_LAUNCH(DT, ENV, RAD) hipLaunchKernelGGL((k_gram_dxdx<DT, ENV, RAD>), dim3(ntiles), dim3(256), 0, s, a, ntiles, bstride)
    if (a.kind) {
        switch (a.D) {
            case 1: DXDX_LAUNCH(1, false, true); break;
            case 2: DXDX_LAUNCH(2, false, true); break;
            case 3: DXDX_LAUNCH(3, false, true); break;
            default: DXDX_LAUNCH(0, false, true); break;
        }
    } else if (env) {
        switch (a.D) {
            case 1: DXDX_LAUNCH(1, true, false); break;
            case 2: DXDX_LAUNCH(2, true, false); break;
            case 3: DXDX_LAUNCH(3, true, false); break;
            default: DXDX_LAUNCH(0, true, false); break;
        }
    } else {
        switch (a.D) {
            case 1: DXDX_LAUNCH(1, false, false); break;
            case 2: DXDX_LAUNCH(2, false, false); break;
            case 3: DXDX_LAUNCH(3, false, false); break;
            default: DXDX_LAUNCH(0, false, false); break;
        }
    }
#undef DXDX_LAUNCH
    if (a.ev1) HIP_TRY(hipEventRecord(a.ev1, s));
    HIP_TRY(hipGetLastError());
    return 0;
}

template <int DM, int N, bool ZG, bool ENV>
__device__ __forceinline__ void moment_term(double* mom, const double (&g)[4][4], const double (&p)[4][DM], const double (&q)[4][DM],
                                            const TileLds<DM>& L, int t, int D,
                                            const double (&cu)[4], const double (&su)[4], const double (&cw)[4], const double (&sw)[4],
                                            double (&zr)[4][DM], double (&zc)[4][DM]) {
    const double* V = L.V[t];
    const double* s = L.s[t];
    const double* Mv = L.M[t];
    const double A = L.A[t];
    double vp[4][DM];
    if (N > 0) {
#pragma unroll
        for (int m = 0; m < 4; ++m)
            for (int d = 0; d < D; ++d) vp[m][d] = L.Kp[t][d] * p[m][d];
    }
#pragma unroll
    for (int m = 0; m < 4; ++m)
#pragma unroll
        for (int n = 0; n < 4; ++n) {
            double u[DM];
            for (int d = 0; d < D; ++d) u[d] = (p[m][d] - q[n][d]) + s[d];
            double e;
            if (N > 0) {
                double z = vp[m][0] * q[n][0];
                for (int d = 1; d < D; ++d) z = fma(vp[m][d], q[n][d], z);
                e = exp_taylor<N>(z);
            } else {
                e = gauss_general<DM>(p[m], q[n], V, s, L.L[t], L.e[t], D);
            }
            const double ge = g[m][n] * e;
            const double kc = ge * fma(cu[m], cw[n], su[m] * sw[n]);
            const double ks = ge * fma(su[m], cw[n], -cu[m] * sw[n]);
            mom[0] += kc;
            mom[1] += ks;
            for (int d = 0; d < D; ++d) {
                const double uk = u[d] * kc;
                mom[2 + d] = fma(u[d], uk, mom[2 + d]);
                mom[2 + D + d] += uk;
                mom[2 + 2 * D + d] = fma(u[d], ks, mom[2 + 2 * D + d]);
                if (ENV) {
                    const double a = 0.5 * (p[m][d] + q[n][d]) + L.e[t][d];
                    const double ak = a * kc;
                    mom[2 + 3 * D + d] = fma(a, ak, mom[2 + 3 * D + d]);
                    mom[2 + 4 * D + d] += ak;
                }
                if (ZG) {
                    const double j = -A * fma(V[d], uk, 6.283185307179586476925286766559 * Mv[d] * ks);
                    zr[m][d] += j;
                    zc[n][d] -= j;
                    if (ENV) {
                        const double je = -0.5 * A * L.L[t][d] * (0.5 * (p[m][d] + q[n][d]) + L.e[t][d]) * kc;
                        zr[m][d] += je;
// ... 434 lines not shown
                for (int off = 16; off > 0; off >>= 1) x += __shfl_xor(x, off, 64);
                if (i == 0) outp[w] = x;
            }
            asm volatile("s_waitcnt lgkmcnt(0)\n\ts_barrier" ::: "memory");
        }
        if (!more) break;
        tile = nxt;
        buf ^= 1;
    }
}

__global__ __launch_bounds__(256) void k_gz_reduce(const double* __restrict__ gzp, int nminor, int D, const int* __restrict__ blk,
                                                   double* __restrict__ out, int64_t ld) {
    const int b = blockIdx.x, pnt = threadIdx.x & 63, part = threadIdx.x >> 6;
    const int first = blk[2 * b], n = blk[2 * b + 1];
    __shared__ double red[4][MOGP_GT], redc[4][MOGP_GT];
    const double* base = gzp + (size_t)b * nminor * D * MOGP_GT;
    for (int d = 0; d < D; ++d) {
        double s = 0.0, c = 0.0;
        for (int k = part; k < nminor; k += 4) {
            const double x = base[((size_t)k * D + d) * MOGP_GT + pnt];
            const double t = s + x;
            c += fabs(s) >= fabs(x) ? (s - t) + x : (x - t) + s;
            s = t;
        }
        __syncthreads();
        red[part][pnt] = s; redc[part][pnt] = c;
        __syncthreads();
        if (part == 0 && pnt < n) {
            double hs = 0.0, hc = 0.0;
#pragma unroll
            for (int q = 0; q < 4; ++q) {
                const double x = red[q][pnt];
                const double t = hs + x;
                hc += fabs(hs) >= fabs(x) ? (hs - t) + x : (x - t) + hs;
                hs = t;
                hc += redc[q][pnt];
            }
            out[(size_t)d * ld + first + pnt] += hs + hc;
        }
    }
}

template <bool DENSE, bool ZG, bool ENV>
static int launch_moments_t(const MomentArgs& a, hipStream_t s) {
    switch (a.D) {
        case 1: hipLaunchKernelGGL((k_moments<1, DENSE, ZG, ENV>), dim3(a.ntiles), dim3(256), 0, s, a); break;
        case 2: hipLaunchKernelGGL((k_moments<2, DENSE, ZG, ENV>), dim3(a.ntiles), dim3(256), 0, s, a); break;
        case 3: hipLaunchKernelGGL((k_moments<3, DENSE, ZG, ENV>), dim3(a.ntiles), dim3(256), 0, s, a); break;
        default: hipLaunchKernelGGL((k_moments<0, DENSE, ZG, ENV>), dim3(a.ntiles), dim3(256), 0, s, a); break;
    }
    HIP_TRY(hipGetLastError());
    return 0;
}

template <bool DENSE>
static void launch_moments_radial(const MomentArgs& a, hipStream_t s, int rows) {
    if (rows == 1) {
        hipLaunchKernelGGL((k_moments<1, DENSE, false, false, true, 1>), dim3(a.ntiles), dim3(256), 0, s, a);
    } else if (rows > 1) {
        switch (a.D) {
            case 1: hipLaunchKernelGGL((k_moments<1, DENSE, false, false, true, 2>), dim3(a.ntiles), dim3(256), 0, s, a); break;
            case 2: hipLaunchKernelGGL((k_moments<2, DENSE, false, false, true, 2>), dim3(a.ntiles), dim3(256), 0, s, a); break;
            case 3: hipLaunchKernelGGL((k_moments<3, DENSE, false, false, true, 2>), dim3(a.ntiles), dim3(256), 0, s, a); break;
            default: hipLaunchKernelGGL((k_moments<0, DENSE, false, false, true, 2>), dim3(a.ntiles), dim3(256), 0, s, a); break;
        }
    } else {
        switch (a.D) {
            case 1: hipLaunchKernelGGL((k_moments<1, DENSE, false, false, true>), dim3(a.ntiles), dim3(256), 0, s, a); break;
            case 2: hipLaunchKernelGGL((k_moments<2, DENSE, false, false, true>), dim3(a.ntiles), dim3(256), 0, s, a); break;
            case 3: hipLaunchKernelGGL((k_moments<3, DENSE, false, false, true>), dim3(a.ntiles), dim3(256), 0, s, a); break;
            default: hipLaunchKernelGGL((k_moments<0, DENSE, false, false, true>), dim3(a.ntiles), dim3(256), 0, s, a); break;
        }
    }
}

int launch_moments(const MomentArgs& a0, hipStream_t s, int rows) {
    if (a0.ntiles <= 0) return 0;
    MomentArgs a = a0;
    if (a.W <= 0) a.W = 2 + 3 * a.D;
    const bool env = a.W > 2 + 3 * a.D;
    const double* xc = a.xc ? a.xc : a.x;
    const int64_t ldxc = a.xc ? a.ldxc : a.ldx;
    int rc = a.phases_ready ? 0 : launch_phase_tables(a.ph, a.x, a.ldx, a.nrows, xc, ldxc, a.xc ? a.ncols : a.nrows, a.table, a.T, a.D, a.C, a.W, s);
    if (rc) return rc;
    if (a.kind) {
        if (!a.shape) { set_error("launch_moments: kinds without shapes"); return -1; }
        if (env || (a.G != nullptr && (!a.sym || a.ru || a.gzr || a.gzc || a.xc))) { set_error("launch_moments: radial profiles take the exact mode or a dense symmetric adjoint, without an envelope"); return -1; }
        if (a.ev0) HIP_TRY(hipEventRecord(a.ev0, s));
        if (rows == 1 && a.D != 1) { set_error("launch_moments: gate rows take one input dimension"); return -1; }
        if (a.G != nullptr) launch_moments_radial<true>(a, s, rows); else launch_moments_radial<false>(a, s, rows);
        HIP_TRY(hipGetLastError());
        if (a.ev1) HIP_TRY(hipEventRecord(a.ev1, s));
        return 0;
    }
    if (a.G == nullptr) {
        if (a.ev0) HIP_TRY(hipEventRecord(a.ev0, s));
        if (!env && a.D == 1 && a.W == 5 && a.T <= 4 && a.row_mod <= 1 && a.xc == nullptr) {
            static const int ncu = []() { int dev = 0; hipDeviceProp_t pr; if (hipGetDevice(&dev) != hipSuccess || hipGetDeviceProperties(&pr, dev) != hipSuccess) return 256; return pr.multiProcessorCount; }();
            if (a.T <= 3) hipLaunchKernelGGL(k_moments_x<3>, dim3(std::min(a.ntiles, ncu)), dim3(512), 0, s, a);
            else hipLaunchKernelGGL(k_moments_x<4>, dim3(std::min(a.ntiles, ncu)), dim3(512), 0, s, a);
            HIP_TRY(hipGetLastError());
            rc = 0;
        } else
        rc = env ? launch_moments_t<false, false, true>(a, s) : launch_moments_t<false, false, false>(a, s);
        if (!rc && a.ev1) HIP_TRY(hipEventRecord(a.ev1, s));
        return rc;
    }
    if (a.gzr || a.gzc) {
        if (!a.gzp || !a.rblk || !a.cblk || a.nrb <= 0 || a.ncb <= 0) { set_error("launch_moments: the input-gradient pass needs its scratch and block tables"); return -1; }
        const size_t half = (size_t)a.nrb * a.ncb * a.D * MOGP_GT;
        HIP_TRY(hipMemsetAsync(a.gzp, 0, 2 * half * sizeof(double), s));
        if ((rc = env ? launch_moments_t<true, true, true>(a, s) : launch_moments_t<true, true, false>(a, s))) return rc;
        if (a.gzr) hipLaunchKernelGGL(k_gz_reduce, dim3(a.nrb), dim3(256), 0, s, a.gzp, a.ncb, a.D, a.rblk, a.gzr, a.ldgz);
        if (a.gzc) hipLaunchKernelGGL(k_gz_reduce, dim3(a.ncb), dim3(256), 0, s, a.gzp + half, a.nrb, a.D, a.cblk, a.gzc, a.ldgz);
        HIP_TRY(hipGetLastError());
        return 0;
    }
    return env ? launch_moments_t<true, false, true>(a, s) : launch_moments_t<true, false, false>(a, s);
}

__global__ __launch_bounds__(256) void k_moment_reduce(const double* __restrict__ partial, const int* __restrict__ pair_start,
                                                       int TW, int W, int D, int lower_pairs, double* __restrict__ out) {
    const int p = blockIdx.x, tw = blockIdx.y;
    const int b = pair_start[p], e = pair_start[p + 1];
    __shared__ double red[256];
    double s = 0.0;
    for (int t = b + threadIdx.x; t < e; t += 256) s += partial[(size_t)t * TW + tw];
    red[threadIdx.x] = s;
    __syncthreads();
    for (int off = 128; off > 0; off >>= 1) {
        if (threadIdx.x < off) red[threadIdx.x] += red[threadIdx.x + off];
        __syncthreads();
    }
    if (threadIdx.x == 0) {
        int i = (int)((sqrt(8.0 * (double)p + 1.0) - 1.0) * 0.5);
        while ((i + 1) * (i + 2) / 2 <= p) ++i;
        while (i * (i + 1) / 2 > p) --i;
        const bool diag = lower_pairs && (p - i * (i + 1) / 2) == i;
        const int w = tw % W;
        double v = red[0];
        if (diag && (w == 1 || (w >= 2 + D && w < 2 + 2 * D))) v = 0.0;
        out[(size_t)p * TW + tw] = v;
    }
}

int launch_moment_reduce(const double* partial, const int* pair_start, int npairs, int T, int W, int D, double* out, hipStream_t s, int lower_pairs) {
    hipLaunchKernelGGL(k_moment_reduce, dim3(npairs, T * W), dim3(256), 0, s, partial, pair_start, T * W, W, D, lower_pairs, out);
    HIP_TRY(hipGetLastError());
    return 0;
}

__global__ void k_diagG(const double* __restrict__ kinv, int64_t ld, const double* __restrict__ alpha,
                        const int* __restrict__ chan_off, double* __restrict__ out, double kinv_sign, int row_mod, int row_rem) {
    const int c = blockIdx.x;
    __shared__ double red[256];
    double s = 0.0;
    for (int64_t k = chan_off[c] + threadIdx.x; k < chan_off[c + 1]; k += 256)
        if (row_mod <= 1 || (int)((k / MOGP_TILE) % row_mod) == row_rem) s += 0.5 * (alpha[k] * alpha[k] - kinv_sign * kinv[k * ld + k]);
    red[threadIdx.x] = s;
    __syncthreads();
    for (int off = 128; off > 0; off >>= 1) {
        if (threadIdx.x < off) red[threadIdx.x] += red[threadIdx.x + off];
        __syncthreads();
    }
    if (threadIdx.x == 0) out[c] = red[0];
}

int launch_diagG(const double* kinv, int64_t ld, const double* alpha, const int* chan_off, int C, double* out, hipStream_t s,
                 double kinv_sign, int row_mod, int row_rem) {
    hipLaunchKernelGGL(k_diagG, dim3(C), dim3(256), 0, s, kinv, ld, alpha, chan_off, out, kinv_sign, row_mod, row_rem);
    HIP_TRY(hipGetLastError());
    return 0;
}

}
```

### mogptk_amd/csrc/mogp_api.hip

```cpp
#include "mogp_model.h"

#include <algorithm>
#include <cmath>
#include <cstring>
#include <cstdlib>

namespace mogp {

static thread_local std::string g_err;
void set_error(const std::string& msg) { g_err = msg; }
int hip_fail(hipError_t e, const char* what, const char* file, int line) {
    g_err = std::string("HIP error '") + hipGetErrorString(e) + "' in " + what + " (" + file + ":" + std::to_string(line) + ")";
    return MOGP_EHIP;
}
int launch_potrf_trtri_tile(double* A, int64_t ld, int t, double* invd, double* logdet, unsigned long long* info, hipStream_t s,
                            long long info_base = 0, int store_L = 0);

int fail(int code, const std::string& msg) { g_err = msg; return code; }

int sort_inputs(const double* X, int64_t M, int D, int C, int64_t pad_to, SortedX& o) {
    o.M = M;
    o.Mpad = round_up(std::max<int64_t>(M, 1), pad_to);
    o.perm.resize(M);
    o.off.assign(C + 1, 0);
// ... 558 lines not shown
        build_sym_tiles(m->sx.off, m->C, m->tiles, m->pair_start);
        if ((rc = m->d_tiles.ensure(m->tiles.size()))) return rc;
        if ((rc = m->d_pair_start.ensure(m->pair_start.size()))) return rc;
        HIP_TRY(dev_upload(m->d_tiles.p, m->tiles.data(), m->tiles.size() * sizeof(GTile)));
        if ((rc = m->strip.build(m->tiles))) return rc;
        for (const GTile& t : m->tiles) (t.c0 < 4 * MOGP_TILE ? m->tiles_head : m->tiles_tail).push_back(t);
        if (!m->tiles_head.empty() && !m->tiles_tail.empty()) {
            if ((rc = m->d_tiles_head.ensure(m->tiles_head.size()))) return rc;
            if ((rc = m->d_tiles_tail.ensure(m->tiles_tail.size()))) return rc;
            HIP_TRY(dev_upload(m->d_tiles_head.p, m->tiles_head.data(), m->tiles_head.size() * sizeof(GTile)));
            HIP_TRY(dev_upload(m->d_tiles_tail.p, m->tiles_tail.data(), m->tiles_tail.size() * sizeof(GTile)));
            if ((rc = m->strip_head.build(m->tiles_head))) return rc;
            if ((rc = m->strip_tail.build(m->tiles_tail))) return rc;
        }
        HIP_TRY(dev_upload(m->d_pair_start.p, m->pair_start.data(), m->pair_start.size() * sizeof(int)));
    }
    if ((rc = m->d_partial.ensure(m->tiles.size() * (size_t)std::max(m->T, 1) * (size_t)std::max(m->Wt, 1)))) return rc;
    if (m->k.Npad == m->Npad) return (m->k.owned_rows && !m->sh_owned) ? spd_make_whole(m->k) : 0;
    return spd_alloc(m->k, m->Npad, m->sh_owned ? m->ctx->device : -1);
} }

extern "C" {

static int ctx_streams(mogp_ctx* ctx) {
    if (ctx->streams_ready) return 0;
    int lo_prio = 0;
    {
        int lo = 0, hi = 0;
        HIP_TRY(hipDeviceGetStreamPriorityRange(&lo, &hi));
        lo_prio = lo;
        HIP_TRY(hipStreamCreateWithPriority(&ctx->st, hipStreamNonBlocking, hi));
        const char* er = std::getenv("MOGP_RESERVE_CUS");
        const int reserve = er ? std::atoi(er) : 2;
        hipDeviceProp_t prop;
        HIP_TRY(hipGetDeviceProperties(&prop, ctx->device));
        const int ncu = prop.multiProcessorCount;
        const bool masked = reserve > 0 && 16 * reserve < ncu;
        ctx->ncu = ncu; ctx->ncu_reserved = masked ? 8 * reserve : 0;
        ctx->chain_ok = !masked || 8 * reserve >= 13;
        if (masked) {
            std::vector<uint32_t> bulk((ncu + 31) / 32, 0u), priv((ncu + 31) / 32, 0u);
            for (int i = 0; i < ncu; ++i) (i < 8 * reserve ? priv : bulk)[i / 32] |= 1u << (i % 32);
            HIP_TRY(hipExtStreamCreateWithCUMask(&ctx->st_priv, (uint32_t)priv.size(), priv.data()));
            HIP_TRY(hipExtStreamCreateWithCUMask(&ctx->st2, (uint32_t)bulk.size(), bulk.data()));
            HIP_TRY(hipExtStreamCreateWithCUMask(&ctx->st3, (uint32_t)bulk.size(), bulk.data()));
            HIP_TRY(hipExtStreamCreateWithCUMask(&ctx->st4, (uint32_t)bulk.size(), bulk.data()));
        } else {
            HIP_TRY(hipStreamCreateWithPriority(&ctx->st2, hipStreamNonBlocking, (lo + hi) / 2));
            HIP_TRY(hipStreamCreateWithPriority(&ctx->st3, hipStreamNonBlocking, lo));
            HIP_TRY(hipStreamCreateWithPriority(&ctx->st4, hipStreamNonBlocking, lo));
        }
    }
    {
        hipDeviceProp_t prop;
        HIP_TRY(hipGetDeviceProperties(&prop, ctx->device));
        std::vector<uint32_t> all((prop.multiProcessorCount + 31) / 32, 0u);
        for (int i = 0; i < prop.multiProcessorCount; ++i) all[i / 32] |= 1u << (i % 32);
        if (ctx->st_priv) HIP_TRY(hipExtStreamCreateWithCUMask(&ctx->st2u, (uint32_t)all.size(), all.data()));
        else HIP_TRY(hipStreamCreateWithPriority(&ctx->st2u, hipStreamNonBlocking, lo_prio));
    }
    ctx->streams_ready = true;
    return 0;
}

int mogp_model_create(mogp_ctx* ctx, int64_t N, int D, int C, const double* X, const double* y, mogp_model** out) {
    if (!ctx || !X || !y || !out) return fail(MOGP_EINVAL, "mogp_model_create: null argument");
    *out = nullptr;
    if (N <= 0 || D <= 0 || D > MOGP_MAXD || C <= 0) return fail(MOGP_EINVAL, "mogp_model_create: need N > 0, 0 < D <= 8, C > 0");
    int rc;
    if ((rc = use_device(ctx))) return rc;
    mogp_model* m = new mogp_model();
    m->ctx = ctx; m->N = N; m->D = D; m->C = C;
    if ((rc = sort_inputs(X, N, D, C, MOGP_TILE, m->sx))) { delete m; return rc; }
    m->Npad = m->sx.Mpad;
    m->nb = (int)(m->Npad / MOGP_TILE);
    const int64_t Npad = m->Npad;
    const int nchunks = (int)((Npad + 511) / 512);
#define TRY_RC(x) do { int r__ = (x); if (r__) { mogp_model_destroy(m); return r__; } } while (0)
#define TRY_HIP(x) do { hipError_t e__ = (x); if (e__ != hipSuccess) { int r__ = hip_fail(e__, #x, __FILE__, __LINE__); mogp_model_destroy(m); return r__; } } while (0)
    TRY_RC(ctx_streams(ctx));
    m->st = ctx->st; m->st2 = ctx->st2; m->st2u = ctx->st2u; m->st3 = ctx->st3; m->st4 = ctx->st4; m->st_priv = ctx->st_priv;
    TRY_RC(m->d_x.ensure((size_t)D * Npad));
    TRY_RC(m->d_y.ensure(Npad));
    TRY_RC(m->d_noise.ensure(C));
    TRY_RC(m->d_z.ensure(Npad));
    TRY_RC(m->d_alpha.ensure((size_t)(1 + nchunks) * Npad));
    TRY_RC(m->d_zz.ensure((Npad + 3) / 4));
    TRY_RC(m->d_diagG.ensure(C));
    TRY_RC(m->d_info.ensure(2));
    TRY_RC(m->d_flag.ensure(1));
    TRY_RC(m->d_chan_off.ensure(C + 1));
    TRY_HIP(dev_upload(m->d_x.p, m->sx.xs.data(), (size_t)D * Npad * sizeof(double)));
    TRY_HIP(dev_upload(m->d_chan_off.p, m->sx.off.data(), (C + 1) * sizeof(int)));
    TRY_RC(mogp_model_set_y(m, y));
#undef TRY_RC
#undef TRY_HIP
    *out = m;
    return MOGP_OK;
}

int mogp_model_destroy(mogp_model* m) {
    if (!m) return MOGP_OK;
    if (m->ctx) { hipError_t e = hipSetDevice(m->ctx->device); (void)e; }
    if (m->st) { hipError_t e = hipStreamSynchronize(m->st); (void)e; }
    for (auto e : m->ev) { hipError_t r = hipEventDestroy(e); (void)r; }
    for (auto e : m->gemm_ev) { hipError_t r = hipEventDestroy(e); (void)r; }
    for (auto& e : m->pred_ev) if (e) { hipError_t r = hipEventDestroy(e); (void)r; e = nullptr; }
    for (hipStream_t q : {m->st2, m->st2u, m->st3, m->st4, m->ctx->st5, m->st_priv}) if (q) { hipError_t e = hipStreamSynchronize(q); (void)e; }
    m->k.release(); m->ws.release(); m->ws_tail.release();
    for (int b = 0; b < 2; ++b) { m->swU[b].release(); m->swUr[b].release(); m->swXr[b].release(); }
    for (auto e : m->sw_ev) { hipError_t r = hipEventDestroy(e); (void)r; }
    for (auto e : m->sh_prof) { hipError_t r = hipEventDestroy(e); (void)r; }
    m->d_symv.release(); m->sh_send.release(); m->sh_recv.release(); m->sh_send1.release(); m->sh_recv1.release(); m->sh_fact.release();
    for (auto e : m->sh_ev) { hipError_t r = hipEventDestroy(e); (void)r; }
    if (m->tw) { m->tw->release(); delete m->tw; m->tw = nullptr; }
    m->oa.release();
    m->loo.release();
    m->cv.release();
    m->d_x.release(); m->d_y.release(); m->d_table.release(); m->d_kind.release(); m->d_shape.release();
    m->d_noise.release(); m->d_dvar.release(); m->d_z.release(); m->d_alpha.release(); m->d_zz.release();
    m->d_partial.release(); m->d_moments.release(); m->d_diagG.release(); m->d_tiles.release(); m->d_pair_start.release(); m->strip.release(); m->strip_own.release();
    m->d_tiles_head.release(); m->d_tiles_tail.release(); m->strip_head.release(); m->strip_tail.release();
    if (m->gram_ev) { hipError_t r = hipEventDestroy(m->gram_ev); (void)r; m->gram_ev = nullptr; }
    if (m->gram_tail_ev) { hipError_t r = hipEventDestroy(m->gram_tail_ev); (void)r; m->gram_tail_ev = nullptr; }
    m->d_chan_off.release(); m->d_flag.release(); m->d_info.release(); m->d_pivots.release(); m->acc_rhs.release();
    m->d_xs.release(); m->d_Ksf.release(); m->d_Vt.release(); m->d_mu.release(); m->d_var.release(); m->d_kdiag.release();
    m->d_Kss.release(); m->d_parts.release(); m->d_ptiles.release(); m->d_pred_tasks.release();
    m->ph_xx.release(); m->ph_sx.release(); m->ph_ss.release();
    if (m->h_pin) { hipError_t e = hipHostFree(m->h_pin); (void)e; m->h_pin = nullptr; }
    mean_release(m);

    delete m;
    return MOGP_OK;
}

int mogp_model_set_y(mogp_model* m, const double* y) {
    if (!m || !y) return fail(MOGP_EINVAL, "mogp_model_set_y: null argument");
    int rc;
    if ((rc = use_device(m->ctx))) return rc;
    std::vector<double> ys(m->Npad, 0.0);
    for (int64_t pos = 0; pos < m->N; ++pos) ys[pos] = y[m->sx.perm[pos]];
    if (m->mean_on) {
        HIP_TRY(dev_upload(m->d_y0.p, ys.data(), m->Npad * sizeof(double)));
        m->hy0 = ys;
        m->mean_g_valid = m->mean_g_pending = false;
        return mean_apply(m);
    }
    HIP_TRY(dev_upload(m->d_y.p, ys.data(), m->Npad * sizeof(double)));
    m->hy = ys;
    return MOGP_OK;
}

int mogp_model_set_terms_ex(mogp_model* m, int T, int width, const double* table) {
    if (!m || !table || T <= 0) return fail(MOGP_EINVAL, "mogp_model_set_terms: bad argument");
    if (width != 2 + 3 * m->D && width != 2 + 5 * m->D) return fail(MOGP_EINVAL, "mogp_model_set_terms: the row width must be 2 + 3 D or 2 + 5 D");
    int rc;
    if ((rc = use_device(m->ctx))) return rc;
    const int W = width;
    const size_t n = (size_t)m->C * m->C * T * W;
    for (size_t i = 0; i < n; ++i)
        if (!std::isfinite(table[i])) return fail(MOGP_ENONFINITE, "spectral term table has non-finite entries (kernel parameters diverged)");
    if (T != m->T) { m->radial = m->point_kinds = false; m->gate_kinds = 0; }
    m->T = T;
    m->Wt = W;
    if (m->tw) m->tw->pred_valid = false;
    m->table.assign(table, table + n);
    if ((rc = m->d_table.ensure(n))) return rc;
    if ((rc = m->d_moments.ensure((size_t)(m->C * (m->C + 1) / 2) * T * W))) return rc;
    HIP_TRY(hipMemcpyAsync(m->d_table.p, m->table.data(), n * sizeof(double), hipMemcpyHostToDevice, m->st));
    return MOGP_OK;
}

int mogp_model_set_terms(mogp_model* m, int T, const double* table) {
    if (!m) return fail(MOGP_EINVAL, "mogp_model_set_terms: bad argument");
    return mogp_model_set_terms_ex(m, T, 2 + 3 * m->D, table);
}

int mogp_model_set_kinds(mogp_model* m, int T, const int* kind, const double* shape) {
    if (!m) return fail(MOGP_EINVAL, "mogp_model_set_kinds: model is null");
    if (T != m->T || T <= 0) return fail(MOGP_EINVAL, "mogp_model_set_kinds: T must be that of the last mogp_model_set_terms");
    const size_t n = (size_t)m->C * m->C * T;
    bool any = false;
    if (const char* bad = check_kinds(kind, shape, m->C, m->D, T, &any)) return fail(MOGP_EINVAL, std::string("mogp_model_set_kinds: ") + bad);
    m->radial = false; m->point_kinds = false; m->gate_kinds = 0;
    if (!any) return MOGP_OK;
    if (m->Wt != 2 + 3 * m->D) return fail(MOGP_EINVAL, "mogp_model_set_kinds: radial profiles do not combine with enveloped term rows");
    m->hkind.assign(kind, kind + n);
    m->hshape.assign(shape, shape + n);
    for (size_t i = 0; i < n; ++i) {
        const int k = kind[i] & MOGP_KIND_MASK;
        m->point_kinds |= k == MOGP_KIND_DOT || k == MOGP_KIND_GATE || k == MOGP_KIND_WDOT;
    }
    m->gate_kinds = extra_rows(kind, n);
    int rc;
    if ((rc = use_device(m->ctx))) return rc;
    if ((rc = m->d_kind.ensure(n))) return rc;
    if ((rc = m->d_shape.ensure(n))) return rc;
    HIP_TRY(hipMemcpyAsync(m->d_kind.p, kind, n * sizeof(int), hipMemcpyHostToDevice, m->st));
    HIP_TRY(hipMemcpyAsync(m->d_shape.p, shape, n * sizeof(double), hipMemcpyHostToDevice, m->st));
    m->radial = true;
    return MOGP_OK;
}

int mogp_model_set_point_diag(mogp_model* m, const double* kdiag) {
    if (!m) return fail(MOGP_EINVAL, "mogp_model_set_point_diag: model is null");
    m->point_diag.clear();
    if (kdiag) {
        m->point_diag.resize(m->N);
        for (int64_t pos = 0; pos < m->N; ++pos) m->point_diag[pos] = kdiag[m->sx.perm[pos]];
    }
    return MOGP_OK;
}

int mogp_gram(mogp_ctx* ctx, int C, int D, int T, const double* table, int64_t M1, const double* X1,
              int64_t M2, const double* X2, double* K_out) {
    return mogp_gram_ex(ctx, C, D, T, 2 + 3 * D, table, M1, X1, M2, X2, K_out);
}

int mogp_gram_ex(mogp_ctx* ctx, int C, int D, int T, int width, const double* table, int64_t M1, const double* X1,
                 int64_t M2, const double* X2, double* K_out) {
    return mogp_gram_kinds(ctx, C, D, T, width, table, nullptr, nullptr, M1, X1, M2, X2, K_out);
}

int mogp_gram_kinds(mogp_ctx* ctx, int C, int D, int T, int width, const double* table, const int* kind, const double* shape,
                    int64_t M1, const double* X1, int64_t M2, const double* X2, double* K_out) {
    if (!ctx || !table || !X1 || !K_out || M1 <= 0 || T <= 0 || C <= 0 || D <= 0 || D > MOGP_MAXD || (width != 2 + 3 * D && width != 2 + 5 * D))
        return fail(MOGP_EINVAL, "mogp_gram: bad argument");
    bool radial = false;
    if (const char* bad = check_kinds(kind, shape, C, D, T, &radial)) return fail(MOGP_EINVAL, std::string("mogp_gram_kinds: ") + bad);
    if (radial && width != 2 + 3 * D) return fail(MOGP_EINVAL, "mogp_gram_kinds: kinds need shapes and rows of width 2 + 3 D");
    int rc;
    if ((rc = use_device(ctx))) return rc;
    const bool sym = (X2 == nullptr);
    SortedX s1, s2;
    if ((rc = sort_inputs(X1, M1, D, C, 1, s1))) return rc;
    if (!sym && (rc = sort_inputs(X2, M2, D, C, 1, s2))) return rc;
    const SortedX& sc = sym ? s1 : s2;
    const int64_t R = s1.M, Cc = sc.M;
    std::vector<GTile> tiles;
    std::vector<int> ps;
    if (sym) build_sym_tiles(s1.off, C, tiles, ps); else build_rect_tiles(s1.off, s2.off, C, tiles);
    const int W = width;
    DevBuf<double> dx1, dx2, dtab, dout;
    DevBuf<GTile> dt;
    DevBuf<int> dkind;
    DevBuf<double> dshape;
    PhaseWs ph;
    auto cleanup = [&]() { dx1.release(); dx2.release(); dtab.release(); dout.release(); dt.release(); dkind.release(); dshape.release(); ph.release(); };
#define G_TRY(x) do { int r__ = (x); if (r__) { cleanup(); return r__; } } while (0)
#define G_HIP(x) do { hipError_t e__ = (x); if (e__ != hipSuccess) { cleanup(); return hip_fail(e__, #x, __FILE__, __LINE__); } } while (0)
    G_TRY(dx1.ensure((size_t)D * s1.Mpad));
// ... 192 lines not shown
```

### mogptk_amd/csrc/mogp_internal.h

```cpp
#pragma once
#include <hip/hip_runtime.h>
#include <stdint.h>
#include <atomic>
#include <string>
#include <vector>

#define MOGP_TILE 128
#define MOGP_GT 64
#define MOGP_TC 8
#define MOGP_MAXD 8

#define MOGP_KIND_GAUSS 0
#define MOGP_KIND_RQ 1
#define MOGP_KIND_MATERN12 2
#define MOGP_KIND_MATERN32 3
#define MOGP_KIND_MATERN52 4
#ifndef MOGP_KIND_PERIODIC
#define MOGP_KIND_PERIODIC 5
#endif
#ifndef MOGP_KIND_SINC
#define MOGP_KIND_SINC 6
#define MOGP_KIND_DOT 7
#define MOGP_DOT_DEGREE_MAX 8
#endif
#ifndef MOGP_KIND_GATE
#define MOGP_KIND_GATE 8
#endif
#ifndef MOGP_KIND_WDOT
#define MOGP_KIND_WDOT 9
#define MOGP_KIND_WHITE 10
#endif
#ifndef MOGP_KIND_TIMES
#define MOGP_KIND_TIMES (1 << 8)
#endif
#define MOGP_KIND_MASK 0xff
#define MOGP_GROUP_MAX 4

namespace mogp {
const char* check_kinds(const int* kind, const double* shape, int C, int D, int T, bool* any);
}

namespace mogp {

void set_error(const std::string& msg);
int hip_fail(hipError_t e, const char* what, const char* file, int line);
#define HIP_TRY(x)                                                        \
    do {                                                                  \
        hipError_t e__ = (x);                                             \
        if (e__ != hipSuccess) return mogp::hip_fail(e__, #x, __FILE__, __LINE__); \
    } while (0)

inline int set_max_dynamic_lds(const void* fn, int bytes, std::atomic<unsigned long long>& done) {
    int dev = 0;
    HIP_TRY(hipGetDevice(&dev));
    const unsigned long long bit = 1ull << (dev & 63);
    if (done.load(std::memory_order_acquire) & bit) return 0;
    HIP_TRY(hipFuncSetAttribute(fn, hipFuncAttributeMaxDynamicSharedMemorySize, bytes));
    done.fetch_or(bit, std::memory_order_release);
    return 0;
}

struct GTile {
    int r0, c0;
    int nr, nc;
    int pair;
    int flags;
    int rb, cb;
};
struct GSeg { int r0, c0, n, pair; int diag, pad[3]; };
enum { GT_MIRROR = 1,
       GT_DIAG = 2 };

struct PhaseRef {
    const int* offr = nullptr;
    const int* offc = nullptr;
    double* ws = nullptr;
};
size_t phase_ws_doubles(int C, int T, int64_t ldr, int64_t ldc);

struct GramArgs {
    const GTile* tiles;
    const double* xr;
    const double* xc;
    int64_t ldxr, ldxc;
    int64_t nrows, ncols;
    PhaseRef ph;
    const double* table;
    int T, D, C;
    int W;
    double* out;
    int64_t ldo;
    double* out2;
    const double* noise;
    const double* dvar;
    double jitter_abs;
    int mirror;
    hipEvent_t ev0, ev1;
    const GSeg* segs; int nsegs;
    const GTile* rest; int nrest;
    int dbg;
    int tab_lds;
    int phases_ready;
    const int* kind;
    const double* shape;
};

struct MomentArgs {
    const GTile* tiles;
    int ntiles;
    const double* x;
    int64_t ldx;
    const double* xc;
    int64_t ldxc;
    int64_t nrows, ncols;
    PhaseRef ph;
    const double* table;
    int T, D, C;
    int W;
    const double* kinv;
    int64_t ld;
    const double* alpha;
    double kinv_sign;
    int row_mod, row_rem;
    const double* G;
    int64_t ldg;
    const double* ru;
    const double* rw;
    double rcoef;
    int sym;
    double* gzr;
    double* gzc;
    int64_t ldgz;
    double* gzp;
    int nrb, ncb;
    const int* rblk;
    const int* cblk;
    double* partial;
    hipEvent_t ev0, ev1;
    int tab_lds;
    int phases_ready;
    const int* kind;
    const double* shape;
};

int launch_gram(const GramArgs& a, int ntiles, hipStream_t s, int rows = 0);
int launch_gram_dx(const GramArgs& a, int ntiles, int64_t dstride, hipStream_t s);
int launch_gram_dxdx(const GramArgs& a, int ntiles, int64_t bstride, hipStream_t s);
void split_strip_tiles(const std::vector<GTile>& tiles, int maxrun, std::vector<GSeg>& segs, std::vector<GTile>& rest);
int launch_moments(const MomentArgs& a, hipStream_t s, int rows = 0);
inline int extra_rows(const int* kind, size_t n) {
    int rows = 0;
    for (size_t i = 0; i < n; ++i) {
        const int k = kind[i] & MOGP_KIND_MASK;
        if (k == MOGP_KIND_WDOT || k == MOGP_KIND_WHITE) return 2;
        if (k == MOGP_KIND_GATE) rows = 1;
    }
    return rows;
}
inline size_t gz_scratch_doubles(int nrb, int ncb, int D) { return (size_t)2 * nrb * ncb * D * MOGP_GT; }
void tile_blocks(const std::vector<int>& off, int C, std::vector<int>& blk);
int launch_moment_reduce(const double* partial, const int* pair_start, int npairs, int T, int W, int D, double* out, hipStream_t s,
                         int lower_pairs = 1);
int launch_diagG(const double* kinv, int64_t ld, const double* alpha, const int* chan_off, int C, double* out, hipStream_t s,
                 double kinv_sign = 1.0, int row_mod = 0, int row_rem = 0);

enum GemmMode { GM_RECT = 0,
                GM_LOWER = 1,
                GM_LAUUM = 2,
                GM_KHI_J = 3,
                GM_TASKS = 4,
                GM_RECT_LOWER = 5,
                GM_KHI_I = 6,
                GM_KLO_J = 7,
                GM_KLO_I = 8 };

struct GemmTask {
    int64_t a_off, b_off, c_off;
    int kt;
    int pad;
};

struct GemmArgs {
    const double* A; int64_t lda; int a_kmajor;
    const double* B; int64_t ldb; int b_kmajor;
    double* C; int64_t ldc;
    double alpha, beta;
    int mode, mt, nt, K;
    const GemmTask* tasks; int ntasks;
    int task_chunked;
    int small;
    int beta0_from;
    int ksplit; int64_t c_split;
    int ksplit_xcd;
    int col_major;
    int row_mod, row_rem, row_off, row_shift;
    int sk_hint;
    int sk_spans;
    double* sk_ws;
    unsigned* sk_flags;
    unsigned sk_epoch;
    unsigned long long* sk_info;
    unsigned* fl_flags; int fl_nwait; unsigned fl_widx[4]; unsigned fl_wval[4];
    int fl_wt, fl_sig; unsigned fl_sig_base; int fl_sig_shift; unsigned* fl_err; unsigned fl_spins; unsigned* fl_diag;
};
int launch_gemm(const GemmArgs& a, hipStream_t s);
double gemm_flops(const GemmArgs& a, const std::vector<GemmTask>* host_tasks);

int launch_potrf_tile(double* A, int64_t ld, int t, double* logdet, unsigned long long* info, hipStream_t s);
int launch_trtri_tiles(const double* A, int64_t ld, int t0, int nt, double* invd, hipStream_t s);
int launch_put_diag_tiles(double* A, int64_t ld, int nt, const double* invd, hipStream_t s);
int launch_wkk(const double* Ablk, int64_t ld, const double* invd, int nk, double* Wk, int64_t ldw, hipStream_t s);
#define MOGP_CHAIN_FLAGS 32
#define MOGP_INFO_CHAIN_TIMEOUT 0ull
struct ChainFlow {
    unsigned* wait_flag; unsigned wait_val;
    unsigned* done_flag;
    int write_through;
    unsigned long long* trace;
    unsigned* diag;
};
int launch_chain(double* A, int64_t ld, int t0, int nk, double* invd, double* logdet, unsigned long long* info, long long info_base,
                 double* Wk, int64_t ldw, unsigned* flags, unsigned* err, hipStream_t s, const ChainFlow* flow = nullptr);

#define FLOW_MAXQ 48
#define FLOW_NCAS 1
#define FLOW_TRACE_W 6
#define FLOW_POST_W 96
#define FLOW_KEY_STEP 1024
#define FLOW_NOSIG 0xffffffffu
struct FlowTask {
    uint16_t ar, ac, br, bc, cr, cc;
    uint8_t abuf, bbuf, cbuf, var;
    uint16_t kt, ndep;
    uint32_t dep[4];
    uint16_t need[4];
    uint32_t sig[2];
    uint32_t key;
    uint32_t pad[2];
};
static_assert(sizeof(FlowTask) == 64, "FlowTask layout");
enum { FLOW_DIAG_DEEP = 0, FLOW_DIAG_HEAD_STALE = 1, FLOW_DIAG_DEP_STALE = 2, FLOW_DIAG_WAIT_DEEP = 3, FLOW_DIAG_WAIT_STALE = 4, FLOW_DIAG_LAST = 5, FLOW_DIAG_WORDS = 8 };
struct FlowPlan {
    int nb = 0, ob = 0, nouter = 0, nq = 0, rhs_nt = 0;
    bool replay = false;
    std::vector<FlowTask> tasks;
    std::vector<FlowTask> folded;
    int qbase[FLOW_MAXQ] = {0}, qsize[FLOW_MAXQ] = {0};
// ... 29 lines not shown
```

### mogptk_amd/csrc/mogp_model.h

```cpp
#pragma once
#include "../../include/mogp_hip.h"
#include "mogp_internal.h"

#include <algorithm>
#include <cmath>
#include <cstring>
#include <string>
#include <map>
#include <vector>

namespace mogp {

inline int dev_fill_zero(void* p, size_t bytes) {
    HIP_TRY(hipMemset(p, 0, bytes));
    HIP_TRY(hipStreamSynchronize(nullptr));
    return 0;
}

inline hipError_t dev_upload(void* dst, const void* src, size_t bytes) {
    hipError_t e = hipMemcpy(dst, src, bytes, hipMemcpyHostToDevice);
    return e != hipSuccess ? e : hipStreamSynchronize(nullptr);
}

template <typename T>
struct DevBuf {
    T* p = nullptr;
    size_t n = 0;
    bool borrowed = false;
    int ensure(size_t count) {
        if (count <= n) return 0;
        if (borrowed) { set_error("DevBuf: a borrowed range cannot grow"); return -1; }
        if (p) { hipError_t e = hipFree(p); (void)e; p = nullptr; n = 0; }
        HIP_TRY(hipMalloc(reinterpret_cast<void**>(&p), count * sizeof(T)));
        n = count;
        return 0;
    }
    void release() { if (p && !borrowed) { hipError_t e = hipFree(p); (void)e; } p = nullptr; n = 0; borrowed = false; }
};

struct RowBacked {
    static constexpr size_t GRAN = (size_t)2 << 20;
    char* base = nullptr;
    size_t bytes = 0, gran = GRAN;
    int device = 0;
    std::vector<hipMemGenericAllocationHandle_t> handle;
    std::vector<char> have;
    size_t nbacked = 0;
    int reserve(size_t nbytes, int dev) {
        release();
        bytes = (nbytes + gran - 1) / gran * gran;
        void* q = nullptr;
        HIP_TRY(hipMemAddressReserve(&q, bytes, gran, nullptr, 0));
        base = static_cast<char*>(q); device = dev;
        have.assign(bytes / gran, 0);
        handle.resize(bytes / gran);
        return 0;
    }
    int back(size_t off, size_t len) {
        if (len == 0) return 0;
        if (!base || off + len > bytes) { set_error("RowBacked::back: outside the reserved range"); return -1; }
        const size_t g_lo = off / gran, g_hi = (off + len - 1) / gran;
        hipMemAllocationProp prop{};
        prop.type = hipMemAllocationTypePinned; prop.location.type = hipMemLocationTypeDevice; prop.location.id = device;
        hipMemAccessDesc acc{};
        acc.location.type = hipMemLocationTypeDevice; acc.location.id = device; acc.flags = hipMemAccessFlagsProtReadWrite;
        for (size_t g = g_lo; g <= g_hi;) {
            if (have[g]) { ++g; continue; }
            size_t e = g;
            for (; e <= g_hi && !have[e]; ++e) {
                HIP_TRY(hipMemCreate(&handle[e], gran, &prop, 0));
                hipError_t me = hipMemMap(base + e * gran, gran, 0, handle[e], 0);
                if (me == hipSuccess) me = hipMemSetAccess(base + e * gran, gran, &acc, 1);
                if (me != hipSuccess) { hipError_t x = hipMemUnmap(base + e * gran, gran); x = hipMemRelease(handle[e]); (void)x; HIP_TRY(me); }
                have[e] = 1; ++nbacked;
            }
            { int z__ = dev_fill_zero(base + g * gran, (e - g) * gran); if (z__) return z__; }
            g = e;
        }
        return 0;
    }
    size_t backed_bytes() const { return nbacked * gran; }
    void release() {
        for (size_t g = 0; g < have.size(); ++g)
            if (have[g]) {
                hipError_t e = hipMemUnmap(base + g * gran, gran); (void)e;
                e = hipMemRelease(handle[g]); (void)e;
            }
        have.clear(); handle.clear(); nbacked = 0;
        if (base) { hipError_t e = hipMemAddressFree(base, bytes); (void)e; }
        base = nullptr; bytes = 0;
    }
};

struct PhaseWs {
    DevBuf<double> ws;
    DevBuf<int> offr, offc;
    std::vector<int> hr, hc;
    int prepare(const std::vector<int>& r, const std::vector<int>& c, int C, int T, int64_t ldr, int64_t ldc, hipStream_t s, PhaseRef& out) {
        int rc;
        if ((rc = ws.ensure(phase_ws_doubles(C, T, ldr, ldc)))) return rc;
        if (hr != r) {
            if ((rc = offr.ensure(r.size()))) return rc;
            hr = r;
            HIP_TRY(hipMemcpyAsync(offr.p, hr.data(), hr.size() * sizeof(int), hipMemcpyHostToDevice, s));
        }
        if (hc != c) {
            if ((rc = offc.ensure(c.size()))) return rc;
            hc = c;
            HIP_TRY(hipMemcpyAsync(offc.p, hc.data(), hc.size() * sizeof(int), hipMemcpyHostToDevice, s));
        }
        out.offr = offr.p; out.offc = offc.p; out.ws = ws.p;
        return 0;
    }
    void release() { ws.release(); offr.release(); offc.release(); hr.clear(); hc.clear(); }
};

struct SortedX {
    int64_t M = 0, Mpad = 0;
    std::vector<int64_t> perm;
    std::vector<int> off;
    std::vector<double> xs;
    bool identity = true;
};


int fail(int code, const std::string& msg);
static inline int64_t round_up(int64_t v, int64_t m) { return (v + m - 1) / m * m; }
int sort_inputs(const double* X, int64_t M, int D, int C, int64_t pad_to, SortedX& o);
void build_sym_tiles(const std::vector<int>& off, int C, std::vector<GTile>& tiles, std::vector<int>& pair_start);
void build_rect_tiles(const std::vector<int>& offr, const std::vector<int>& offc, int C, std::vector<GTile>& tiles,
                      std::vector<int>* pair_start = nullptr);

}

using namespace mogp;

enum { MOGP_COMM_NONE = 0, MOGP_COMM_RCCL = 1, MOGP_COMM_EXTERNAL = 2 };
struct mogp_comm {
    int kind = MOGP_COMM_NONE, rank = 0, n = 1;
    void* nccl = nullptr;
    mogp_allgather_cb allgather = nullptr;
    mogp_allreduce_cb allreduce = nullptr;
    void* user = nullptr;
};

struct mogp_ctx {
    int device = 0;
    mogp_comm comm;
    std::string name;
    hipStream_t st = nullptr, st2 = nullptr, st3 = nullptr, st4 = nullptr, st5 = nullptr, st_priv = nullptr, st2u = nullptr;
    bool streams_ready = false;
    bool chain_ok = true;
    struct SkWs { DevBuf<double> ws; DevBuf<unsigned> flags; unsigned epoch = 0; };
    std::map<hipStream_t, SkWs> sk;
    int ncu = 0, ncu_reserved = 0;
};

struct TrtriLevel {
    std::vector<GemmTask> h1, h2;
    DevBuf<GemmTask> d1, d2;
    double flops1 = 0, flops2 = 0;
};

#define MOGP_CHAIN_BOUND_TILES 160
#define MOGP_OUTER 4
#define MOGP_NPANEL 4
struct Spd {
    int64_t Npad = 0;
    int nb = 0;
    bool keep_L = false;
    bool refine_panels = false;
    DevBuf<double> pscr;
    DevBuf<double> A, B, invd, logdet;
    RowBacked Arows;
    bool owned_rows = false;
    DevBuf<double> Wm;
    std::vector<TrtriLevel> levels;
    std::vector<hipEvent_t> sync_ev;
    std::vector<hipEvent_t> row_ev;
    bool want_row_ev = false;
    std::vector<hipEvent_t> inv_ev;
    hipEvent_t fused_last_inv = nullptr, fused_last_wt = nullptr;
    DevBuf<double> Wd;
    DevBuf<double> Pb[MOGP_NPANEL];
    DevBuf<unsigned> chain_flags;
    DevBuf<double> Lm, Wt;
    FlowPlan flow;
    DevBuf<FlowTask> flow_tasks;
    DevBuf<int> flow_qmeta;
    FlowPlan flow_replay;
    DevBuf<FlowTask> flow_tasks_replay;
    DevBuf<int> flow_qmeta_replay;
    FlowPlan flow_rhs;
    DevBuf<FlowTask> flow_tasks_rhs;
    DevBuf<int> flow_qmeta_rhs;
    const FlowPlan* flow_cur = nullptr;
    DevBuf<unsigned> flow_flags;
// ... 100 lines not shown
};

struct FlowRhs { double* T; double* X; int nt; hipEvent_t ready; };
struct mogp_model {
    mogp_ctx* ctx = nullptr;
    int64_t N = 0, Npad = 0;
    int nb = 0, D = 0, C = 0, T = 0;
    int Wt = 0;
    std::vector<double> point_diag;
    SortedX sx;
    std::vector<GTile> tiles;
    std::vector<int> pair_start;
    std::vector<double> table;
    int gate_kinds = 0;
    bool radial = false;
    mogp::DevBuf<int> d_kind;
    std::vector<int> hkind;
    mogp::DevBuf<double> d_shape;
    std::vector<double> hshape;
    bool point_kinds = false;
    hipStream_t st = nullptr;
    hipStream_t st2 = nullptr;
    hipStream_t st2u = nullptr;
    hipStream_t st3 = nullptr;
    hipStream_t st4 = nullptr;
    hipStream_t st_priv = nullptr;
    Spd k;
    Spd ws, ws_tail;
    DevBuf<double> swU[2], swUr[2];
    DevBuf<double> swXr[2];
    std::vector<hipEvent_t> sw_ev;
    int sh_rank = 0, sh_n = 1;
    bool sh_owned = false;
    int backed_rank = -1, backed_n = 0;
    std::vector<GTile> tiles_own;
    std::vector<int> pair_start_own;
    DevBuf<GTile> d_tiles_own;
    bool factor_only = false;
    hipEvent_t pred_ev[2] = {nullptr, nullptr};
    StripTiles strip, strip_own;
    std::vector<GTile> tiles_head, tiles_tail;
    DevBuf<GTile> d_tiles_head, d_tiles_tail;
    StripTiles strip_head, strip_tail;
    hipEvent_t gram_ev = nullptr, gram_tail_ev = nullptr;
    DevBuf<int> d_pair_start_own;
    int own_rank = -1, own_n = 0;
    DevBuf<double> sh_send, sh_recv;
    DevBuf<double> sh_send1, sh_recv1;
    DevBuf<double> sh_fact;
    bool sh_factor_once = false;
    bool sh_split = false;
    std::vector<hipEvent_t> sh_ev;
    std::vector<hipEvent_t> sh_prof;
    double sh_ms[6] = {0, 0, 0, 0, 0, 0};
    int sh_prof_blocks = 0;
    double sh_jabs = 0.0;
    bool sh_dvar = false;

    std::vector<double> hy;
    DevBuf<double> d_symv;
    DevBuf<double> d_x, d_y, d_table, d_noise, d_dvar, d_z, d_alpha, d_zz, d_partial, d_moments, d_diagG;
    DevBuf<GTile> d_tiles;
    std::vector<GemmTask> kinv_acc_tasks, kinv_lauum_tasks;
    std::vector<int> kinv_prefix;
    DevBuf<GemmTask> d_kinv_acc, d_kinv_lauum;
    std::vector<double> blk_cen, blk_half;
    bool kinv_sparse = false;
    double kinv_fraction = 1.0;
    DevBuf<int> d_pair_start, d_chan_off, d_flag;
    DevBuf<double> d_pivots;
    bool accurate = false, accurate_ran = false;
    DevBuf<double> acc_rhs;
    double pivot_min = 0.0, pivot_max = 0.0;
    DevBuf<unsigned long long> d_info;

    DevBuf<double> d_xs, d_Ksf, d_Vt, d_mu, d_var, d_kdiag, d_Kss;
    DevBuf<double> d_parts;
    DevBuf<GTile> d_ptiles;
    DevBuf<GemmTask> d_pred_tasks;
    PhaseWs ph_xx, ph_sx, ph_ss;

    double* h_pin = nullptr;
    size_t h_pin_n = 0;

    bool profiling = false;
    std::vector<hipEvent_t> ev;
    std::vector<hipEvent_t> gemm_ev;
    size_t gemm_ev_used = 0;
    double ms[MOGP_ST_COUNT] = {0};
    int64_t gemm_launches = 0;
    double gemm_flops = 0.0;
    bool have_W = false, have_Kinv = false, kinv_in_A = false, w_in_Wm = false;
    bool flow_ran = false;
    const FlowRhs* rhs_job = nullptr;
    bool replay_flow = false;
    bool no_flow = false;
    long long n_fact = 0, flow_retry_at = 0;
    int flow_backoff = 64, flow_timeouts = 0;
    double flow_enqueue_us = 0.0, flow_enqueue_us_max = 0.0;
    bool no_chain = false;
    TitsiasWork* tw = nullptr;
    OaWork oa;
    LooWork loo;
    CvWork cv;

    bool mean_on = false, mean_g_valid = false, mean_g_pending = false;
    std::vector<double> mean_coef, mean_g, hy0;
    DevBuf<double> d_y0, d_mean_coef, d_mean_part, d_mean_g;
    double* h_mean_pin = nullptr;
    hipEvent_t mean_ev = nullptr;
    const double* mean_w = nullptr;
    double mean_w_scale = 0.0;
};


namespace mogp {
int use_device(mogp_ctx* c);
int gemm_call(mogp_model* m, const GemmArgs& g, double flops, hipStream_t st = nullptr);
int mark(mogp_model* m, int idx);
double table_diag(const mogp_model* m, int c);
double table_diag_points(const mogp_model* m, const SortedX& pts);
int mean_apply(mogp_model* m);
int mean_grad_enqueue(mogp_model* m, const double* w, double scale);
void mean_grad_collect(mogp_model* m);
void mean_release(mogp_model* m);
int spd_alloc(Spd& w, int64_t Npad, int owned_rows_device = -1);
int spd_make_whole(Spd& w);
inline GemmArgs make_gemm(const double* A, int64_t lda, int akm, const double* B, int64_t ldb, int bkm, double* C, int64_t ldc,
                          double alpha, int mode, int mt, int nt, int64_t K) {
    GemmArgs g{};
    g.A = A; g.lda = lda; g.a_kmajor = akm; g.B = B; g.ldb = ldb; g.b_kmajor = bkm; g.C = C; g.ldc = ldc;
    g.alpha = alpha; g.beta = 0.0; g.mode = mode; g.mt = mt; g.nt = nt; g.K = (int)K;
    return g;
}
int side_fork(mogp_model* m, TitsiasWork& t, hipStream_t* side);
int side_join(mogp_model* m, TitsiasWork& t, hipStream_t side);
int gz_prepare(mogp_model* m, TitsiasWork& t, const std::vector<int>& offz, int D);
void gz_attach(const TitsiasWork& t, MomentArgs& ma, bool zx);
int spd_check_info(mogp_model* m, const char* which, int64_t* info);
int spd_info_verdict(mogp_model* m, const char* which, unsigned long long hinfo, int64_t* info);
int sparse_timeout_check(mogp_model* m);
bool chain_enabled(const mogp_model* m);
int chain_fallback(mogp_model* m);
int spd_invert(mogp_model* m, Spd& w, const char* which, int64_t* info, const double** W, bool defer_check = false);
int mm_lower_splitk(mogp_model* m, TitsiasWork& t, const double* A, const double* B, double* out, int mt, int64_t Mpad, int64_t ldk, int64_t K,
                    double alpha = 1.0);
int launch_scale_cols(const double* in, double* out, int64_t ld, int64_t rows, int64_t n, const double* s, hipStream_t st);
int sparse_workspace(mogp_model* m, TitsiasWork& t, int64_t Mpad, int64_t M);
int sparse_tiles(mogp_model* m, TitsiasWork& t, const SortedX& sz, bool want_uf);
int sparse_kuu(mogp_model* m, int64_t M, const double* Z, double jitter, bool want_uf, SortedX& sz, double* jit, const char* need_grouped = nullptr);
int sparse_kuf(mogp_model* m, TitsiasWork& t, const SortedX& sz, hipStream_t stream, bool use_strips, double* out2);
int refined_apply(mogp_model* m, TitsiasWork& t, const double* P, const double* Q, const double* rhs, double* out);
int allreduce_vec_scalars(mogp_model* m, TitsiasWork& t, double* vec, int64_t n, double* hs, int k);
int adjoint_GA(mogp_model* m, TitsiasWork& t, double scale, hipStream_t stream);
int solve_with_rider(mogp_model* m, TitsiasWork& t, double* panel, const double* r, double* beta);
struct MomentSpec { const double* G; int64_t ldg; const double* ru; const double* rw; double rcoef; bool dz; };
int sparse_moments(mogp_model* m, TitsiasWork& t, const SortedX& sz, const MomentSpec* uf, const MomentSpec& uu, bool sharded, hipStream_t side);
int sparse_predict_panels(mogp_model* m, TitsiasWork& t, const SortedX& sz, int64_t S, const double* Xs, SortedX& ss);
int sparse_point_stats(mogp_model* m, TitsiasWork& t, const SortedX& pts, const double* a, const double* b, const double* mu_panel,
                       const double* mu_vec, double mu_div, const double* kdiag, double* mu, double* var);
int sparse_predict_finish(mogp_model* m, TitsiasWork& t, const SortedX& ss, const double* mu_panel, const double* mu_vec, double mu_div,
                          const double* kss_diag, double* mu, double* var);
#define MOGP_RETRY_NO_CHAIN 0x7e7e
int begin_call(mogp_model* m, int64_t* info, bool one_gpu);
int exact_begin(mogp_model* m, const double* noise_var, const double* data_var, double jitter, GramArgs& ga, double& jabs);
int report_not_pd(unsigned long long hinfo, int64_t* info);
// ... 45 lines not shown
```

### mogptk_amd/csrc/shard.hip

```cpp
#include "mogp_model.h"
#include <cstdlib>
#include <limits>

using namespace mogp;

static int sweep_eval_begin(mogp_model* m, const double* noise_var, const double* data_var, double jitter) {
    const int64_t N = m->N, Npad = m->Npad;
    GramArgs ga{};
    int rc = exact_begin(m, noise_var, data_var, jitter, ga, m->sh_jabs);
    if (rc) return rc;
    m->sh_dvar = data_var != nullptr;
    if (m->radial) return fail(MOGP_EINVAL, "the sweep / sharded evaluation does not take radial kinds (mogp_model_set_kinds)");
    const bool own = m->sh_n > 1 && m->own_n == m->sh_n && m->own_rank == m->sh_rank;
    if (own) ga.tiles = m->d_tiles_own.p;
    (own ? m->strip_own : m->strip).attach(ga);
    if ((rc = launch_gram(ga, (int)(own ? m->tiles_own.size() : m->tiles.size()), m->st))) return rc;
    if (!(m->sh_owned && m->sh_n > 1 && (m->nb - 1) % m->sh_n != m->sh_rank))
        if ((rc = launch_pad_identity(m->k.A.p, Npad, N, Npad, m->st))) return rc;
    return mark(m, 1);
}

static int sweep_eval_alpha(mogp_model* m) {
    const int64_t Npad = m->Npad;
    int rc;
    if ((rc = mark(m, 2))) return rc;
    if ((rc = mark(m, 3))) return rc;
    const int nchunks = (int)((Npad + 511) / 512);
    if ((rc = m->d_symv.ensure((size_t)(4 + nchunks) * Npad))) return rc;
    const int rm = m->sh_n > 1 ? m->sh_n : 0;
    if ((rc = launch_symv_lower(m->k.A.p, Npad, Npad, m->d_y.p, m->d_alpha.p, m->d_symv.p, -1.0, m->st, rm, m->sh_rank))) return rc;
    return mark(m, 4);
}

static int sweep_eval_scalars(mogp_model* m, double* lml, int64_t* info) {
    const int64_t N = m->N, Npad = m->Npad;
    const int nb = m->nb;
    const unsigned long long big = std::numeric_limits<unsigned long long>::max();
    std::vector<double> hl(nb), ha(Npad);
    unsigned long long hinfo = 0;
    HIP_TRY(hipMemcpyAsync(hl.data(), m->k.logdet.p, nb * sizeof(double), hipMemcpyDeviceToHost, m->st));
    HIP_TRY(hipMemcpyAsync(ha.data(), m->d_alpha.p, Npad * sizeof(double), hipMemcpyDeviceToHost, m->st));
    HIP_TRY(hipMemcpyAsync(&hinfo, m->d_info.p, sizeof(hinfo), hipMemcpyDeviceToHost, m->st));
    HIP_TRY(hipStreamSynchronize(m->st));
    if (hinfo == MOGP_INFO_CHAIN_TIMEOUT) return MOGP_RETRY_NO_CHAIN;
    if (hinfo != big) return report_not_pd(hinfo, info);
    double logdet = 0.0, ya = 0.0;
    for (double v : hl) logdet += v;
    for (int64_t i = 0; i < N; ++i) ya += m->hy[i] * ha[i];
    if (lml) *lml = -0.5 * (double)N * std::log(2.0 * M_PI) - logdet - 0.5 * ya;
    return 0;
}

namespace mogp { int eval_sweep(mogp_model* m, const double* noise_var, const double* data_var, double jitter, double* lml, double* jitter_abs, int64_t* info) {
    int rc;
    if ((rc = sweep_eval_begin(m, noise_var, data_var, jitter))) return rc;
    if (jitter_abs) *jitter_abs = m->sh_jabs;
    if ((rc = spd_sweep(m, m->k))) return rc;
    if ((rc = sweep_eval_alpha(m))) return rc;
    return sweep_eval_scalars(m, lml, info);
} }

extern "C" {

static int sharded_rc(mogp_model* m, int rc) {
    if (rc != MOGP_RETRY_NO_CHAIN) return rc;
    if ((rc = chain_fallback(m))) return rc;
    return fail(MOGP_EHIP, "chain kernel: a hand-off timed out inside a sharded evaluation; this rank uses the launch-per-step chain from now on -- repeat the call on every rank");
}

int mogp_shard_config(mogp_model* m, int rank, int nranks) {
    if (!m || nranks < 1 || rank < 0 || rank >= nranks) return fail(MOGP_EINVAL, "mogp_shard_config: bad argument");
    m->sh_rank = rank; m->sh_n = nranks;
    static const int owned_mode = []() { const char* e = std::getenv("MOGP_SHARD_OWNED"); return e ? std::atoi(e) : 1; }();
    m->sh_owned = (owned_mode >= 1 && nranks > 1) || owned_mode >= 2;
    { int r__ = use_device(m->ctx); if (r__) return r__; r__ = ensure_system(m); if (r__) return r__; }
    if (nranks > 1 && (m->own_rank != rank || m->own_n != nranks)) {
        int rc;
        if ((rc = use_device(m->ctx))) return rc;
        m->tiles_own.clear();
        m->pair_start_own.assign(1, 0);
        for (size_t p = 0; p + 1 < m->pair_start.size(); ++p) {
            for (int t = m->pair_start[p]; t < m->pair_start[p + 1]; ++t) {
                const GTile& g = m->tiles[t];
                const int a = g.r0 / MOGP_TILE, b = (g.r0 + g.nr - 1) / MOGP_TILE;
                if (a % nranks == rank || b % nranks == rank) m->tiles_own.push_back(g);
            }
            m->pair_start_own.push_back((int)m->tiles_own.size());
        }
        if ((rc = m->d_tiles_own.ensure(std::max<size_t>(m->tiles_own.size(), 1)))) return rc;
        if ((rc = m->d_pair_start_own.ensure(m->pair_start_own.size()))) return rc;
        HIP_TRY(dev_upload(m->d_tiles_own.p, m->tiles_own.data(), m->tiles_own.size() * sizeof(GTile)));
        if ((rc = m->strip_own.build(m->tiles_own))) return rc;
        HIP_TRY(dev_upload(m->d_pair_start_own.p, m->pair_start_own.data(), m->pair_start_own.size() * sizeof(int)));
        m->own_rank = rank; m->own_n = nranks;
    }
    if (m->k.owned_rows && (m->backed_rank != rank || m->backed_n != nranks)) {
        int rc;
        const size_t row_bytes = (size_t)m->Npad * sizeof(double);
        for (int i = rank; i < m->nb; i += nranks)
// ... 259 lines not shown
```

Baseline: 98.39.

## Cut per-evaluation launches and copies by merging small kernels, memsets and transfers

```diff
diff --git a/mogptk_amd/csrc/exact.hip b/mogptk_amd/csrc/exact.hip
--- a/mogptk_amd/csrc/exact.hip
+++ b/mogptk_amd/csrc/exact.hip
@@ -146,14 +146,17 @@
         HIP_TRY(hipMemcpyAsync(m->d_dvar.p, dv.data(), Npad * sizeof(double), hipMemcpyHostToDevice, m->st));
     }
     jabs = jitter * dsum / (double)N;
-    HIP_TRY(hipMemcpyAsync(m->d_noise.p, noise_var, C * sizeof(double), hipMemcpyHostToDevice, m->st));
     static const unsigned long long big = std::numeric_limits<unsigned long long>::max();
-    HIP_TRY(hipMemcpyAsync(m->d_info.p, &big, sizeof(big), hipMemcpyHostToDevice, m->st));
+    m->h_head.resize((size_t)C + 1);
+    std::memcpy(m->h_head.data(), noise_var, C * sizeof(double));
+    std::memcpy(m->h_head.data() + C, &big, sizeof(big));
+    HIP_TRY(hipMemcpyAsync(m->d_noise.p, m->h_head.data(), ((size_t)C + 1) * sizeof(double), hipMemcpyHostToDevice, m->st));
     int rc;
     if ((rc = mark(m, 0))) return rc;
     ga = GramArgs{};
     ga.tiles = m->d_tiles.p; ga.xr = m->d_x.p; ga.xc = m->d_x.p; ga.ldxr = ga.ldxc = Npad; ga.nrows = ga.ncols = N;
     if ((rc = m->ph_xx.prepare(m->sx.off, m->sx.off, C, m->T, Npad, Npad, m->st, ga.ph))) return rc;
+    ga.phases_ready = m->ph_xx.centres_valid ? MOGP_PH_CENTRES : MOGP_PH_NONE;
     ga.table = m->d_table.p; ga.T = m->T; ga.D = m->D; ga.C = C; ga.W = m->Wt;
     ga.out = m->k.A.p; ga.ldo = Npad; ga.noise = m->d_noise.p; ga.dvar = data_var ? m->d_dvar.p : nullptr;
     ga.jitter_abs = jabs; ga.mirror = 0;
@@ -256,6 +259,7 @@
         gh.tiles = m->d_tiles_head.p; m->strip_head.attach(gh); gh.ev1 = nullptr;
         gt.tiles = m->d_tiles_tail.p; m->strip_tail.attach(gt); gt.ev0 = nullptr; gt.phases_ready = 1;
         if ((rc = launch_gram(gh, (int)m->tiles_head.size(), m->st, m->radial ? m->gate_kinds : 0))) return rc;
+        m->ph_xx.centres_valid = true;
         if ((rc = launch_pad_identity(m->k.A.p, Npad, N, Npad, m->st))) return rc;
         if (!m->gram_ev) HIP_TRY(hipEventCreateWithFlags(&m->gram_ev, hipEventDisableTiming));
         HIP_TRY(hipEventRecord(m->gram_ev, m->st));
@@ -266,6 +270,7 @@
         m->k.tail_ready = m->gram_tail_ev;
     } else {
         if ((rc = launch_gram(ga, (int)m->tiles.size(), m->st, m->radial ? m->gate_kinds : 0))) return rc;
+        m->ph_xx.centres_valid = true;
         if ((rc = launch_pad_identity(m->k.A.p, Npad, N, Npad, m->st))) return rc;
     }
     ga.ev0 = ga.ev1 = nullptr;
@@ -389,8 +394,8 @@
     ma.phases_ready = 1;
     ma.ev0 = prof_event(m, 9); ma.ev1 = prof_event(m, 10);
     if ((rc = launch_moments(ma, m->st, m->radial ? m->gate_kinds : 0))) return rc;
-    if ((rc = launch_moment_reduce(m->d_partial.p, own ? m->d_pair_start_own.p : m->d_pair_start.p, P, T, W, D, m->d_moments.p, m->st))) return rc;
-    if ((rc = launch_diagG(kinv, Npad, m->d_alpha.p, m->d_chan_off.p, C, m->d_diagG.p, m->st, ksign, rm, m->sh_rank))) return rc;
+    if ((rc = launch_moment_tail(m->d_partial.p, own ? m->d_pair_start_own.p : m->d_pair_start.p, P, T, W, D, m->d_moments.p,
+                                 kinv, Npad, m->d_alpha.p, m->d_chan_off.p, C, m->d_diagG.p, m->st, ksign, rm, m->sh_rank))) return rc;
     if ((rc = mean_grad_enqueue(m, m->d_alpha.p, -1.0))) return rc;
     return mark(m, 6);
 }
@@ -463,8 +468,8 @@
 }
 
 static int grad_enqueue(mogp_model* m, const PinLayout& pl) {
-    HIP_TRY(hipMemcpyAsync(m->h_pin + pl.moments, m->d_moments.p, (pl.diagG - pl.moments) * sizeof(double), hipMemcpyDeviceToHost, m->st));
-    HIP_TRY(hipMemcpyAsync(m->h_pin + pl.diagG, m->d_diagG.p, m->C * sizeof(double), hipMemcpyDeviceToHost, m->st));
+    if (m->d_diagG.p != m->d_moments.p + (pl.diagG - pl.moments)) return fail(MOGP_EINVAL, "grad_enqueue: the gradient block does not match the term table's shape");
+    HIP_TRY(hipMemcpyAsync(m->h_pin + pl.moments, m->d_moments.p, (pl.pivots - pl.moments) * sizeof(double), hipMemcpyDeviceToHost, m->st));
     return 0;
 }
 static void grad_finish(mogp_model* m, const double* diagG, double* trG) {
diff --git a/mogptk_amd/csrc/flow.hip b/mogptk_amd/csrc/flow.hip
--- a/mogptk_amd/csrc/flow.hip
+++ b/mogptk_amd/csrc/flow.hip
@@ -726,7 +726,8 @@
         HIP_TRY(dev_upload(d_tasks.p, plan.tasks.data(), plan.tasks.size() * sizeof(FlowTask)));
         HIP_TRY(dev_upload(d_qmeta.p, qm, sizeof(qm)));
     }
-    if ((rc = w.flow_flags.ensure((size_t)plan.nflags))) return rc;
+    const size_t chain_at = ((size_t)plan.nflags + 63) / 64 * 64, nzero = chain_at + (size_t)plan.nouter * MOGP_CHAIN_FLAGS;
+    if ((rc = w.flow_flags.ensure(nzero))) return rc;
     if (!w.flow_diag.p) {
         if ((rc = w.flow_diag.ensure(FLOW_DIAG_WORDS))) return rc;
         HIP_TRY(hipMemsetAsync(w.flow_diag.p, 0, FLOW_DIAG_WORDS * sizeof(unsigned), crit));
@@ -734,9 +735,8 @@
     w.flow_cur = &plan;
     const FlowPlan& p = plan;
     const int nouter = p.nouter;
-    if ((rc = w.chain_flags.ensure((size_t)(nouter + 1) * MOGP_CHAIN_FLAGS))) return rc;
-    HIP_TRY(hipMemsetAsync(w.chain_flags.p, 0, (size_t)(nouter + 1) * MOGP_CHAIN_FLAGS * sizeof(unsigned), crit));
-    HIP_TRY(hipMemsetAsync(w.flow_flags.p, 0, (size_t)p.nflags * sizeof(unsigned), crit));
+    unsigned* const chain_flags = w.flow_flags.p + chain_at;
+    HIP_TRY(hipMemsetAsync(w.flow_flags.p, 0, nzero * sizeof(unsigned), crit));
     if (replay) {
         std::vector<unsigned> preset((size_t)p.nflags, 0u);
         for (const FlowPlan::Chain& c : p.chain) preset[c.done_idx] = c.expect;
@@ -839,7 +839,7 @@
         cf.trace = want_trace ? w.flow_trace.p + FLOW_TRACE_W * p.tasks.size() + 4 * (size_t)kb : nullptr;
         cf.diag = w.flow_diag.p;
         if ((rc = launch_chain(w.A.p, ld, k0, nk, w.invd.p, w.logdet.p, m->d_info.p, 0, w.Wm.p + (int64_t)k0 * MOGP_TILE * (ld + 1), ld,
-                               w.chain_flags.p + (size_t)kb * MOGP_CHAIN_FLAGS, ferr, priv, &cf))) return rc;
+                               chain_flags + (size_t)kb * MOGP_CHAIN_FLAGS, ferr, priv, &cf))) return rc;
         if (na <= 0) continue;
         GemmArgs t1{};
         t1.A = w.A.p + (int64_t)k1 * MOGP_TILE * ld + (int64_t)k0 * MOGP_TILE; t1.lda = ld; t1.a_kmajor = 0;
diff --git a/mogptk_amd/csrc/gram.hip b/mogptk_amd/csrc/gram.hip
--- a/mogptk_amd/csrc/gram.hip
+++ b/mogptk_amd/csrc/gram.hip
@@ -58,25 +58,27 @@
 
 struct PhaseArgs {
     const double* x; int64_t ld; const int* off; const double* table; int T, D, C, W, role; double* cs; double* sn;
+    double* cs1; double* sn1;
 };
 __global__ __launch_bounds__(256) void k_phase_table(PhaseArgs a) {
     const int64_t pt = (int64_t)blockIdx.x * 256 + threadIdx.x;
     if (pt >= a.off[a.C]) return;
-    const int o = blockIdx.y, t = blockIdx.z, D = a.D, W = a.W;
+    const int role = a.role < 0 ? (int)blockIdx.z / a.T : a.role;
+    const int o = blockIdx.y, t = a.role < 0 ? (int)blockIdx.z % a.T : (int)blockIdx.z, D = a.D, W = a.W;
     int c = 0;
     while (pt >= a.off[c + 1]) ++c;
-    const int pair = a.role == 0 ? c * a.C + o : o * a.C + c;
+    const int pair = role == 0 ? c * a.C + o : o * a.C + c;
     const double* row = a.table + ((size_t)pair * a.T + t) * W;
-    double ph = a.role == 0 ? row[1] : 0.0;
+    double ph = role == 0 ? row[1] : 0.0;
     for (int d = 0; d < D; ++d) {
         const double m = row[2 + D + d], xv = a.x[(size_t)d * a.ld + pt];
-        ph = a.role == 0 ? fma(m, xv + row[2 + 2 * D + d], ph) : fma(m, xv, ph);
+        ph = role == 0 ? fma(m, xv + row[2 + 2 * D + d], ph) : fma(m, xv, ph);
     }
     double sn, cs;
     sincospi(2.0 * frac_turn(ph), &sn, &cs);
     const size_t idx = ((size_t)o * a.T + t) * a.ld + pt;
-    a.cs[idx] = cs;
-    a.sn[idx] = sn;
+    (role == 0 || a.role >= 0 ? a.cs : a.cs1)[idx] = cs;
+    (role == 0 || a.role >= 0 ? a.sn : a.sn1)[idx] = sn;
 }
 
 struct CentreArgs { const double* x; int64_t ld; const int* off; int C, D; double* cen; double* half; };
@@ -106,29 +108,37 @@
 __host__ __device__ static inline PhaseView phase_view(double* ws, int C, int T, int D, int64_t ldr, int64_t ldc) {
     PhaseView v;
     double* p = ws;
+    v.rcen = p; p += (size_t)D * ldr; v.rhalf = p; p += (size_t)D * ldr;
+    v.ccen = p; p += (size_t)D * ldc; v.chalf = p; p += (size_t)D * ldc;
     v.rcs = p; p += (size_t)C * T * ldr; v.rsn = p; p += (size_t)C * T * ldr;
-    v.ccs = p; p += (size_t)C * T * ldc; v.csn = p; p += (size_t)C * T * ldc;
-    v.rcen = p; p += (size_t)D * ldr; v.rhalf = p; p += (size_t)D * ldr;
-    v.ccen = p; p += (size_t)D * ldc; v.chalf = p;
+    v.ccs = p; p += (size_t)C * T * ldc; v.csn = p;
     return v;
 }
 
 static int launch_phase_tables(const PhaseRef& ph, const double* xr, int64_t ldxr, int64_t nr, const double* xc, int64_t ldxc, int64_t nc,
-                               const double* table, int T, int D, int C, int W, hipStream_t s) {
+                               const double* table, int T, int D, int C, int W, hipStream_t s, bool centres_ready = false) {
     if (!ph.ws || !ph.offr || !ph.offc) { set_error("Gram / moment launch without a phase workspace"); return -1; }
     const PhaseView v = phase_view(ph.ws, C, T, D, ldxr, ldxc);
     PhaseArgs a;
     a.table = table; a.T = T; a.D = D; a.C = C; a.W = W;
     a.x = xr; a.ld = ldxr; a.off = ph.offr; a.role = 0; a.cs = const_cast<double*>(v.rcs); a.sn = const_cast<double*>(v.rsn);
-    if (nr > 0) hipLaunchKernelGGL(k_phase_table, dim3((unsigned)((nr + 255) / 256), C, T), dim3(256), 0, s, a);
-    a.x = xc; a.ld = ldxc; a.off = ph.offc; a.role = 1; a.cs = const_cast<double*>(v.ccs); a.sn = const_cast<double*>(v.csn);
-    if (nc > 0) hipLaunchKernelGGL(k_phase_table, dim3((unsigned)((nc + 255) / 256), C, T), dim3(256), 0, s, a);
-    CentreArgs c;
-    c.C = C; c.D = D;
-    c.x = xr; c.ld = ldxr; c.off = ph.offr; c.cen = const_cast<double*>(v.rcen); c.half = const_cast<double*>(v.rhalf);
-    if (nr > 0) hipLaunchKernelGGL(k_block_centres, dim3((unsigned)((nr + MOGP_GT - 1) / MOGP_GT + C)), dim3(64), 0, s, c);
-    c.x = xc; c.ld = ldxc; c.off = ph.offc; c.cen = const_cast<double*>(v.ccen); c.half = const_cast<double*>(v.chalf);
-    if (nc > 0) hipLaunchKernelGGL(k_block_centres, dim3((unsigned)((nc + MOGP_GT - 1) / MOGP_GT + C)), dim3(64), 0, s, c);
+    a.cs1 = const_cast<double*>(v.ccs); a.sn1 = const_cast<double*>(v.csn);
+    if (xr == xc && ldxr == ldxc && nr == nc && ph.offr == ph.offc && nr > 0 && 2 * T <= 65535) {
+        a.role = -1;
+        hipLaunchKernelGGL(k_phase_table, dim3((unsigned)((nr + 255) / 256), C, 2 * T), dim3(256), 0, s, a);
+    } else {
+        if (nr > 0) hipLaunchKernelGGL(k_phase_table, dim3((unsigned)((nr + 255) / 256), C, T), dim3(256), 0, s, a);
+        a.x = xc; a.ld = ldxc; a.off = ph.offc; a.role = 1; a.cs = const_cast<double*>(v.ccs); a.sn = const_cast<double*>(v.csn);
+        if (nc > 0) hipLaunchKernelGGL(k_phase_table, dim3((unsigned)((nc + 255) / 256), C, T), dim3(256), 0, s, a);
+    }
+    if (!centres_ready) {
+        CentreArgs c;
+        c.C = C; c.D = D;
+        c.x = xr; c.ld = ldxr; c.off = ph.offr; c.cen = const_cast<double*>(v.rcen); c.half = const_cast<double*>(v.rhalf);
+        if (nr > 0) hipLaunchKernelGGL(k_block_centres, dim3((unsigned)((nr + MOGP_GT - 1) / MOGP_GT + C)), dim3(64), 0, s, c);
+        c.x = xc; c.ld = ldxc; c.off = ph.offc; c.cen = const_cast<double*>(v.ccen); c.half = const_cast<double*>(v.chalf);
+        if (nc > 0) hipLaunchKernelGGL(k_block_centres, dim3((unsigned)((nc + MOGP_GT - 1) / MOGP_GT + C)), dim3(64), 0, s, c);
+    }
     HIP_TRY(hipGetLastError());
     return 0;
 }
@@ -975,7 +985,7 @@
 #else
     a.dbg = 0;
 #endif
-    int rc = a.phases_ready ? 0 : launch_phase_tables(a.ph, a.xr, a.ldxr, a.nrows, a.xc, a.ldxc, a.ncols, a.table, a.T, a.D, a.C, a.W, s);
+    int rc = a.phases_ready == MOGP_PH_ALL ? 0 : launch_phase_tables(a.ph, a.xr, a.ldxr, a.nrows, a.xc, a.ldxc, a.ncols, a.table, a.T, a.D, a.C, a.W, s, a.phases_ready == MOGP_PH_CENTRES);
     if (rc) return rc;
     static const int ncu = []() { int dev = 0; hipDeviceProp_t pr; if (hipGetDevice(&dev) != hipSuccess || hipGetDeviceProperties(&pr, dev) != hipSuccess) return 256; return pr.multiProcessorCount; }();
     const int grid = std::min(ntiles, 2 * ncu);
@@ -1223,7 +1233,7 @@
     const bool env = a.W > 2 + 3 * a.D;
     if (a.kind && (!a.shape || env)) { set_error("launch_gram_dx: kinds without shapes, or with enveloped term rows"); return -1; }
     if (a.W != 2 + 3 * a.D && a.W != 2 + 5 * a.D) { set_error("launch_gram_dx: table rows of an unknown width"); return -1; }
-    int rc = a.phases_ready ? 0 : launch_phase_tables(a.ph, a.xr, a.ldxr, a.nrows, a.xc, a.ldxc, a.ncols, a.table, a.T, a.D, a.C, a.W, s);
+    int rc = a.phases_ready == MOGP_PH_ALL ? 0 : launch_phase_tables(a.ph, a.xr, a.ldxr, a.nrows, a.xc, a.ldxc, a.ncols, a.table, a.T, a.D, a.C, a.W, s, a.phases_ready == MOGP_PH_CENTRES);
     if (rc) return rc;
     if (a.ev0) HIP_TRY(hipEventRecord(a.ev0, s));
 #define DX_LAUNCH(DT, ENV, RAD) hipLaunchKernelGGL((k_gram_dx<DT, ENV, RAD>), dim3(ntiles), dim3(256), 0, s, a, ntiles, dstride)
@@ -1535,7 +1545,7 @@
     if (a.kind && (!a.shape || env)) { set_error("launch_gram_dxdx: kinds without shapes, or with enveloped term rows"); return -1; }
     if (a.W != 2 + 3 * a.D && a.W != 2 + 5 * a.D) { set_error("launch_gram_dxdx: table rows of an unknown width"); return -1; }
     if (a.xc != a.xr || a.ldxc != a.ldxr || a.ldo < a.D * bstride) { set_error("launch_gram_dxdx: not a symmetric launch, or the output is too narrow for D blocks"); return -1; }
-    int rc = a.phases_ready ? 0 : launch_phase_tables(a.ph, a.xr, a.ldxr, a.nrows, a.xc, a.ldxc, a.ncols, a.table, a.T, a.D, a.C, a.W, s);
+    int rc = a.phases_ready == MOGP_PH_ALL ? 0 : launch_phase_tables(a.ph, a.xr, a.ldxr, a.nrows, a.xc, a.ldxc, a.ncols, a.table, a.T, a.D, a.C, a.W, s, a.phases_ready == MOGP_PH_CENTRES);
     if (rc) return rc;
     if (a.ev0) HIP_TRY(hipEventRecord(a.ev0, s));
 #define DXDX_LAUNCH(DT, ENV, RAD) hipLaunchKernelGGL((k_gram_dxdx<DT, ENV, RAD>), dim3(ntiles), dim3(256), 0, s, a, ntiles, bstride)
@@ -2136,7 +2146,7 @@
     const bool env = a.W > 2 + 3 * a.D;
     const double* xc = a.xc ? a.xc : a.x;
     const int64_t ldxc = a.xc ? a.ldxc : a.ldx;
-    int rc = a.phases_ready ? 0 : launch_phase_tables(a.ph, a.x, a.ldx, a.nrows, xc, ldxc, a.xc ? a.ncols : a.nrows, a.table, a.T, a.D, a.C, a.W, s);
+    int rc = a.phases_ready == MOGP_PH_ALL ? 0 : launch_phase_tables(a.ph, a.x, a.ldx, a.nrows, xc, ldxc, a.xc ? a.ncols : a.nrows, a.table, a.T, a.D, a.C, a.W, s, a.phases_ready == MOGP_PH_CENTRES);
     if (rc) return rc;
     if (a.kind) {
         if (!a.shape) { set_error("launch_moments: kinds without shapes"); return -1; }
@@ -2174,11 +2184,9 @@
     return env ? launch_moments_t<true, false, true>(a, s) : launch_moments_t<true, false, false>(a, s);
 }
 
-__global__ __launch_bounds__(256) void k_moment_reduce(const double* __restrict__ partial, const int* __restrict__ pair_start,
-                                                       int TW, int W, int D, int lower_pairs, double* __restrict__ out) {
-    const int p = blockIdx.x, tw = blockIdx.y;
+__device__ __forceinline__ void moment_reduce_body(const double* __restrict__ partial, const int* __restrict__ pair_start, int p, int tw,
+                                                   int TW, int W, int D, int lower_pairs, double* __restrict__ out, double* red) {
     const int b = pair_start[p], e = pair_start[p + 1];
-    __shared__ double red[256];
     double s = 0.0;
     for (int t = b + threadIdx.x; t < e; t += 256) s += partial[(size_t)t * TW + tw];
     red[threadIdx.x] = s;
@@ -2198,6 +2206,11 @@
         out[(size_t)p * TW + tw] = v;
     }
 }
+__global__ __launch_bounds__(256) void k_moment_reduce(const double* __restrict__ partial, const int* __restrict__ pair_start,
+                                                       int TW, int W, int D, int lower_pairs, double* __restrict__ out) {
+    __shared__ double red[256];
+    moment_reduce_body(partial, pair_start, blockIdx.x, blockIdx.y, TW, W, D, lower_pairs, out, red);
+}
 
 int launch_moment_reduce(const double* partial, const int* pair_start, int npairs, int T, int W, int D, double* out, hipStream_t s, int lower_pairs) {
     hipLaunchKernelGGL(k_moment_reduce, dim3(npairs, T * W), dim3(256), 0, s, partial, pair_start, T * W, W, D, lower_pairs, out);
@@ -2205,10 +2218,8 @@
     return 0;
 }
 
-__global__ void k_diagG(const double* __restrict__ kinv, int64_t ld, const double* __restrict__ alpha,
-                        const int* __restrict__ chan_off, double* __restrict__ out, double kinv_sign, int row_mod, int row_rem) {
-    const int c = blockIdx.x;
-    __shared__ double red[256];
+__device__ __forceinline__ void diagG_body(const double* __restrict__ kinv, int64_t ld, const double* __restrict__ alpha, const int* __restrict__ chan_off,
+                                           int c, double* __restrict__ out, double kinv_sign, int row_mod, int row_rem, double* red) {
     double s = 0.0;
     for (int64_t k = chan_off[c] + threadIdx.x; k < chan_off[c + 1]; k += 256)
         if (row_mod <= 1 || (int)((k / MOGP_TILE) % row_mod) == row_rem) s += 0.5 * (alpha[k] * alpha[k] - kinv_sign * kinv[k * ld + k]);
@@ -2220,6 +2231,11 @@
     }
     if (threadIdx.x == 0) out[c] = red[0];
 }
+__global__ __launch_bounds__(256) void k_diagG(const double* __restrict__ kinv, int64_t ld, const double* __restrict__ alpha,
+                                               const int* __restrict__ chan_off, double* __restrict__ out, double kinv_sign, int row_mod, int row_rem) {
+    __shared__ double red[256];
+    diagG_body(kinv, ld, alpha, chan_off, blockIdx.x, out, kinv_sign, row_mod, row_rem, red);
+}
 
 int launch_diagG(const double* kinv, int64_t ld, const double* alpha, const int* chan_off, int C, double* out, hipStream_t s,
                  double kinv_sign, int row_mod, int row_rem) {
@@ -2228,4 +2244,26 @@
     return 0;
 }
 
-}
+struct MomentTailArgs {
+    const double* partial; const int* pair_start; int nred, TW, W, D, lower_pairs; double* moments;
+    const double* kinv; int64_t ld; const double* alpha; const int* chan_off; double* diag; double kinv_sign; int row_mod, row_rem;
+};
+__global__ __launch_bounds__(256) void k_moment_tail(MomentTailArgs a) {
+    __shared__ double red[256];
+    const int blk = blockIdx.x;
+    if (blk < a.nred) moment_reduce_body(a.partial, a.pair_start, blk / a.TW, blk % a.TW, a.TW, a.W, a.D, a.lower_pairs, a.moments, red);
+    else diagG_body(a.kinv, a.ld, a.alpha, a.chan_off, blk - a.nred, a.diag, a.kinv_sign, a.row_mod, a.row_rem, red);
+}
+
+int launch_moment_tail(const double* partial, const int* pair_start, int npairs, int T, int W, int D, double* moments,
+                       const double* kinv, int64_t ld, const double* alpha, const int* chan_off, int C, double* diag, hipStream_t s,
+                       double kinv_sign, int row_mod, int row_rem) {
+    MomentTailArgs a;
+    a.partial = partial; a.pair_start = pair_start; a.nred = npairs * T * W; a.TW = T * W; a.W = W; a.D = D; a.lower_pairs = 1; a.moments = moments;
+    a.kinv = kinv; a.ld = ld; a.alpha = alpha; a.chan_off = chan_off; a.diag = diag; a.kinv_sign = kinv_sign; a.row_mod = row_mod; a.row_rem = row_rem;
+    hipLaunchKernelGGL(k_moment_tail, dim3((unsigned)(a.nred + C)), dim3(256), 0, s, a);
+    HIP_TRY(hipGetLastError());
+    return 0;
+}
+
+}
diff --git a/mogptk_amd/csrc/mogp_api.hip b/mogptk_amd/csrc/mogp_api.hip
--- a/mogptk_amd/csrc/mogp_api.hip
+++ b/mogptk_amd/csrc/mogp_api.hip
@@ -664,12 +664,11 @@
     m->st = ctx->st; m->st2 = ctx->st2; m->st2u = ctx->st2u; m->st3 = ctx->st3; m->st4 = ctx->st4; m->st_priv = ctx->st_priv;
     TRY_RC(m->d_x.ensure((size_t)D * Npad));
     TRY_RC(m->d_y.ensure(Npad));
-    TRY_RC(m->d_noise.ensure(C));
+    TRY_RC(m->d_noise.ensure((size_t)C + 2));
+    m->d_info.p = reinterpret_cast<unsigned long long*>(m->d_noise.p + C); m->d_info.n = 2; m->d_info.borrowed = true;
     TRY_RC(m->d_z.ensure(Npad));
     TRY_RC(m->d_alpha.ensure((size_t)(1 + nchunks) * Npad));
     TRY_RC(m->d_zz.ensure((Npad + 3) / 4));
-    TRY_RC(m->d_diagG.ensure(C));
-    TRY_RC(m->d_info.ensure(2));
     TRY_RC(m->d_flag.ensure(1));
     TRY_RC(m->d_chan_off.ensure(C + 1));
     TRY_HIP(dev_upload(m->d_x.p, m->sx.xs.data(), (size_t)D * Npad * sizeof(double)));
@@ -748,7 +747,9 @@
     if (m->tw) m->tw->pred_valid = false;
     m->table.assign(table, table + n);
     if ((rc = m->d_table.ensure(n))) return rc;
-    if ((rc = m->d_moments.ensure((size_t)(m->C * (m->C + 1) / 2) * T * W))) return rc;
+    const size_t nmom = (size_t)(m->C * (m->C + 1) / 2) * T * W;
+    if ((rc = m->d_moments.ensure(nmom + m->C))) return rc;
+    m->d_diagG.p = m->d_moments.p + nmom; m->d_diagG.n = (size_t)m->C; m->d_diagG.borrowed = true;
     HIP_TRY(hipMemcpyAsync(m->d_table.p, m->table.data(), n * sizeof(double), hipMemcpyHostToDevice, m->st));
     return MOGP_OK;
 }
diff --git a/mogptk_amd/csrc/mogp_internal.h b/mogptk_amd/csrc/mogp_internal.h
--- a/mogptk_amd/csrc/mogp_internal.h
+++ b/mogptk_amd/csrc/mogp_internal.h
@@ -77,6 +77,9 @@
     double* ws = nullptr;
 };
 size_t phase_ws_doubles(int C, int T, int64_t ldr, int64_t ldc);
+enum { MOGP_PH_NONE = 0,
+       MOGP_PH_ALL = 1,
+       MOGP_PH_CENTRES = 2 };
 
 struct GramArgs {
     const GTile* tiles;
@@ -163,6 +166,9 @@
                          int lower_pairs = 1);
 int launch_diagG(const double* kinv, int64_t ld, const double* alpha, const int* chan_off, int C, double* out, hipStream_t s,
                  double kinv_sign = 1.0, int row_mod = 0, int row_rem = 0);
+int launch_moment_tail(const double* partial, const int* pair_start, int npairs, int T, int W, int D, double* moments,
+                       const double* kinv, int64_t ld, const double* alpha, const int* chan_off, int C, double* diag, hipStream_t s,
+                       double kinv_sign = 1.0, int row_mod = 0, int row_rem = 0);
 
 enum GemmMode { GM_RECT = 0,
                 GM_LOWER = 1,
diff --git a/mogptk_amd/csrc/mogp_model.h b/mogptk_amd/csrc/mogp_model.h
--- a/mogptk_amd/csrc/mogp_model.h
+++ b/mogptk_amd/csrc/mogp_model.h
@@ -96,23 +96,28 @@
     DevBuf<double> ws;
     DevBuf<int> offr, offc;
     std::vector<int> hr, hc;
+    bool centres_valid = false;
     int prepare(const std::vector<int>& r, const std::vector<int>& c, int C, int T, int64_t ldr, int64_t ldc, hipStream_t s, PhaseRef& out) {
         int rc;
-        if ((rc = ws.ensure(phase_ws_doubles(C, T, ldr, ldc)))) return rc;
+        const size_t need = phase_ws_doubles(C, T, ldr, ldc);
+        if (need > ws.n) centres_valid = false;
+        if ((rc = ws.ensure(need))) return rc;
         if (hr != r) {
+            centres_valid = false;
             if ((rc = offr.ensure(r.size()))) return rc;
             hr = r;
             HIP_TRY(hipMemcpyAsync(offr.p, hr.data(), hr.size() * sizeof(int), hipMemcpyHostToDevice, s));
         }
         if (hc != c) {
+            centres_valid = false;
             if ((rc = offc.ensure(c.size()))) return rc;
             hc = c;
             HIP_TRY(hipMemcpyAsync(offc.p, hc.data(), hc.size() * sizeof(int), hipMemcpyHostToDevice, s));
         }
-        out.offr = offr.p; out.offc = offc.p; out.ws = ws.p;
+        out.offr = offr.p; out.offc = hr == hc ? offr.p : offc.p; out.ws = ws.p;
         return 0;
     }
-    void release() { ws.release(); offr.release(); offc.release(); hr.clear(); hc.clear(); }
+    void release() { ws.release(); offr.release(); offc.release(); hr.clear(); hc.clear(); centres_valid = false; }
 };
 
 struct SortedX {
@@ -379,6 +384,7 @@
 
     double* h_pin = nullptr;
     size_t h_pin_n = 0;
+    std::vector<double> h_head;
 
     bool profiling = false;
     std::vector<hipEvent_t> ev;
diff --git a/mogptk_amd/csrc/shard.hip b/mogptk_amd/csrc/shard.hip
--- a/mogptk_amd/csrc/shard.hip
+++ b/mogptk_amd/csrc/shard.hip
@@ -15,6 +15,7 @@
     if (own) ga.tiles = m->d_tiles_own.p;
     (own ? m->strip_own : m->strip).attach(ga);
     if ((rc = launch_gram(ga, (int)(own ? m->tiles_own.size() : m->tiles.size()), m->st))) return rc;
+    m->ph_xx.centres_valid = true;
     if (!(m->sh_owned && m->sh_n > 1 && (m->nb - 1) % m->sh_n != m->sh_rank))
         if ((rc = launch_pad_identity(m->k.A.p, Npad, N, Npad, m->st))) return rc;
     return mark(m, 1);
```

Result: no change. 98.56, median of 6 (+0.2%).
